# stevenrobertson/cuburn

Measured on AMD Instinct MI355X. Metric: Msamples/s into 1920x1080 histogram + DE-filter GB/s vs HBM roofline, higher is better.
Workload: dtype f32; 1 GPU; BASELINE configs[1]: 1920x1080 still, 3 xforms (linear+spherical+swirl), 2^28 samples/frame, filters yuv+bilateral+logscale+colorclip, rgba8 out; walker_waves=4, walker_slots=1024, temporal_samples=1024, samples_per_frame=268435456, accum=binned, fuse=256, nslots=1024, frames_queued_ahead=2, frames_per_gpu=1121, parallelism=frame-sharded x1, RCCL gather of device frames, 4 frames per collective

## Files before the change

cuburn_amd/_lib.py:

```python
import ctypes as C
import os

_HERE = os.path.dirname(os.path.abspath(__file__))
LIB_PATH = os.path.join(_HERE, '_lib', 'libflame_hip.so')
LIB_PATH = os.environ.get('FLAME_HIP_LIB', LIB_PATH)

(FL_OK, FL_E_INVAL, FL_E_NOMEM, FL_E_HIP, FL_E_NODEV, FL_E_UNSUPPORTED) = (0, -1, -2, -3, -4, -5)

FILT = dict(yuv=0, bilateral=1, logscale=2, colorclip=3, smearclip=4, haloclip=5, plainclip=6, logencode=7, de=8)
BUF = dict(front=0, back=1, params=2, palette=3, points=4, seeds=5, atom=6, hot=7, side=8)
ACCUM_ATOMIC, ACCUM_BINNED = 0, 1
FL_OP_OPACITY = 10
OUT = dict(rgba8=0, rgba16=1, yuv444p=2, yuv444p10=3, yuv420p10=4, yuv444p12=5)


class fl_dim(C.Structure):
    _fields_ = [(n, C.c_uint32) for n in ('w', 'h', 'aw', 'ah', 'astride')]


_SIGS = {
    'fl_abi_version': (C.c_int, []),
    'fl_last_error': (C.c_char_p, []),
    'fl_calc_dim': (None, [C.c_uint32, C.c_uint32, C.POINTER(fl_dim)]),
    'fl_ctx_create': (C.c_int, [C.c_int, C.c_void_p, C.c_void_p, C.c_uint32, C.c_uint32, C.POINTER(C.c_void_p)]),
    'fl_ctx_destroy': (None, [C.c_void_p]),
    'fl_ctx_sync': (C.c_int, [C.c_void_p]),
    'fl_genome_create': (C.c_int, [C.c_void_p, C.c_void_p, C.c_uint32, C.c_void_p, C.c_uint32, C.c_uint32,
                                   C.POINTER(C.c_void_p)]),
    'fl_genome_destroy': (None, [C.c_void_p]),
    'fl_genome_upload': (C.c_int, [C.c_void_p, C.c_void_p, C.c_void_p, C.c_void_p, C.c_void_p, C.c_void_p, C.c_uint32]),
    'fl_interp': (C.c_int, [C.c_void_p, C.c_void_p, C.c_uint32, C.c_uint32, C.c_float, C.c_float]),
    'fl_iterate': (C.c_int, [C.c_void_p, C.c_void_p, C.c_uint32, C.c_uint32, C.c_double, C.c_uint32, C.c_int,
                             C.POINTER(C.c_uint64)]),
    'fl_filter': (C.c_int, [C.c_void_p, C.c_int, C.c_uint32, C.c_uint32, C.c_void_p, C.c_uint32]),
    'fl_output': (C.c_int, [C.c_void_p, C.c_uint32, C.c_uint32, C.c_int, C.c_void_p, C.c_uint64]),
    'fl_output_bytes': (C.c_size_t, [C.c_uint32, C.c_uint32, C.c_int]),
    'fl_sort_u32': (C.c_int, [C.c_void_p, C.c_uint64, C.c_uint64, C.c_uint32, C.c_uint32, C.c_uint32, C.c_int, C.c_void_p]),
    'fl_frame_begin': (C.c_int, [C.c_void_p, C.POINTER(C.c_uint32)]),
    'fl_frame_ms': (C.c_int, [C.c_void_p, C.c_uint32, C.POINTER(C.c_float)]),
    'fl_frame_query': (C.c_int, [C.c_void_p, C.c_uint32]),
    'fl_host_alloc': (C.c_void_p, [C.c_size_t]),
    'fl_host_free': (None, [C.c_void_p]),
    'fl_timings_reset': (C.c_int, [C.c_void_p]),
    'fl_timings': (C.c_int, [C.c_void_p, C.POINTER(C.c_float), C.POINTER(C.c_float), C.POINTER(C.c_float),
                             C.POINTER(C.c_uint32)]),
    'fl_timings_detail': (C.c_int, [C.c_void_p, C.POINTER(C.c_float * 6)]),
    'fl_launch_stats': (C.c_int, [C.c_void_p, C.POINTER(C.c_uint32 * 4)]),
    'fl_measure_copy': (C.c_int, [C.c_int, C.c_size_t, C.c_int, C.POINTER(C.c_float)]),
    'fl_read_buffer': (C.c_int, [C.c_void_p, C.c_void_p, C.c_int, C.c_void_p, C.c_size_t]),
    'fl_write_buffer': (C.c_int, [C.c_void_p, C.c_void_p, C.c_int, C.c_void_p, C.c_size_t]),
    'fl_buffer_ptr': (C.c_int, [C.c_void_p, C.c_void_p, C.c_int, C.POINTER(C.c_void_p), C.POINTER(C.c_size_t)]),
    'fl_buffer_ptr_async': (C.c_int, [C.c_void_p, C.c_void_p, C.c_int, C.POINTER(C.c_void_p), C.POINTER(C.c_size_t)]),
    'fl_stream_dependency': (C.c_int, [C.c_void_p, C.c_void_p, C.c_int]),
    'fl_reserve': (C.c_int, [C.c_void_p, C.c_uint32, C.c_uint32]),
    'fl_debug_iter_launch': (C.c_int, [C.c_void_p, C.c_void_p, C.c_uint32, C.c_uint32, C.c_uint32, C.c_uint32,
                                       C.c_uint32, C.c_int]),
    'fl_debug_flush': (C.c_int, [C.c_void_p, C.c_uint32, C.c_uint32]),
    'fl_debug_clear': (C.c_int, [C.c_void_p, C.c_uint32, C.c_uint32, C.c_int]),
    'fl_debug_clear_hot': (C.c_int, [C.c_void_p, C.c_uint32, C.c_uint32]),
    'fl_debug_shuffle': (C.c_int, [C.c_void_p, C.c_uint32, C.c_void_p]),
    'fl_debug_counters': (C.c_int, [C.c_void_p, C.c_void_p]),
    'fl_rtc_compile_check': (C.c_int, [C.c_void_p, C.c_uint32, C.c_void_p, C.c_uint32, C.c_int, C.c_int, C.c_int, C.c_char_p, C.c_size_t]),
    'fl_debug_apply_xf': (C.c_int, [C.c_void_p, C.c_void_p, C.c_uint32, C.c_int, C.c_uint32, C.c_void_p, C.c_void_p]),
}
EXPORTS = sorted(_SIGS)

_lib = None


class FlameError(RuntimeError):
    pass


def load():
    global _lib
    if _lib is not None:
        return _lib
    if not os.path.isfile(LIB_PATH):
        raise FlameError('%s not found: build it with `python __graft_entry__.py` '
                         '(make -C cuburn_amd/csrc); the HIP library is required' % LIB_PATH)
    try:
        import torch
    except Exception:
        pass
    lib = C.CDLL(LIB_PATH, mode=C.RTLD_GLOBAL)
    for name, (res, args) in _SIGS.items():
        fn = getattr(lib, name)
        fn.restype, fn.argtypes = res, args
    if lib.fl_abi_version() != 1:
        raise FlameError('libflame_hip ABI mismatch')
    _lib = lib
    return lib


def check(rc):
    if rc == FL_OK:
        return
    msg = load().fl_last_error().decode('utf-8', 'replace')
    if rc == FL_E_NOMEM:
        raise MemoryError(msg)
    if rc in (FL_E_INVAL, FL_E_UNSUPPORTED):
        raise ValueError(msg)
    raise FlameError(msg)
```

cuburn_amd/csrc/flame_abi.hip:

```cpp
#include <hip/hip_runtime.h>
#include <cstdio>
#include <cstdlib>
#include <cstring>
#include <cmath>
#include <string>
#include <atomic>
#include <vector>
#include <algorithm>
#include "kernels.h"
#include "flame_device.h"

static thread_local std::string g_err;
static int fail(int code, const char *what, const char *file, int line, hipError_t e = hipSuccess)
{
    char buf[512];
    if (e != hipSuccess) snprintf(buf, sizeof buf, "%s: %s (%s:%d)", what, hipGetErrorString(e), file, line);
    else snprintf(buf, sizeof buf, "%s (%s:%d)", what, file, line);
    g_err = buf;
    return code;
}
#define HIPCHK(x) do { hipError_t e_ = (x); if (e_ != hipSuccess) \
    return fail(e_ == hipErrorOutOfMemory ? FL_E_NOMEM : FL_E_HIP, #x, __FILE__, __LINE__, e_); } while (0)
#define REQUIRE(c, msg) do { if (!(c)) return fail(FL_E_INVAL, msg, __FILE__, __LINE__); } while (0)

struct EvPair { hipEvent_t a, b; };

struct Lane {
    hipStream_t stream = nullptr;
    size_t nbins = 0;
    float4 *d_front = nullptr, *d_back = nullptr, *d_side = nullptr;
    float *d_blur = nullptr;
    u64 *d_atom = nullptr;
    uint32_t *d_hot = nullptr;
    void *d_outpix = nullptr;
    uint32_t *d_de_tmax = nullptr;
    float *d_de_sinv = nullptr;
    size_t outpix_bytes = 0;
    uint32_t *d_log[2] = {nullptr, nullptr}, *d_dir[2] = {nullptr, nullptr};
    size_t log_words[2] = {0, 0}, dir_words[2] = {0, 0};
    hipStream_t aux = nullptr;
    hipEvent_t ev_it[2] = {nullptr, nullptr}, ev_ac[2] = {nullptr, nullptr};
    float *d_params = nullptr;
    uint64_t params_serial = 0;
    size_t params_floats = 0;
    u64 *d_palette = nullptr;
    hipEvent_t ev_interp_done = nullptr;
    hipEvent_t ev_iter_done = nullptr;
    hipEvent_t ev_out_done = nullptr;
    bool interp_rec = false, iter_rec = false, out_rec = false;
    bool pend_yuv = false, pend_finish = false, pend_log = false;
    float pend_k1 = 0.0f, pend_k2 = 0.0f;
    int pend_in_mode = 0;
    float pend_dp[5] = {0, 0, 0, 0, 0}, pend_k7[7] = {0, 0, 0, 0, 0, 0, 0};
    fl_dim pend_dim = {0, 0, 0, 0, 0};
};

struct fl_ctx {
    int device = 0;
    bool own_stream = false;
    static const int kMaxLanes = 4;
    int nlanes = 2, cur = 0;
    Lane lanes[kMaxLanes];
    uint32_t nslots = 0, nwalkers = 0;
    uint32_t sub_log2 = 0;
    uint32_t ntemporal() const { return nslots << sub_log2; }
    int nw = 4;
    fl_mwc *d_rng = nullptr;
    float4 *d_points = nullptr;
    u64 *d_counters = nullptr;
    uint32_t *d_sort = nullptr; size_t sort_words = 0;
    uint32_t bin_rounds = 16, bin_parts = 0;
    uint32_t launch_rounds = 0;
    uint32_t round_counter = 0;
    static const uint32_t kFrames = 8;
    hipEvent_t ev_begin_[kFrames] = {}, ev_end_[kFrames] = {};
    uint32_t frame_lane[kFrames] = {};
    uint32_t frame_seq = 0;
    std::vector<EvPair> pool, iter_ev, accum_ev, flush_ev, filt_ev, de_ev;
    size_t pool_used = 0;
    bool timing = true;
    static const uint32_t kDepEvents = 16;
    hipEvent_t dep_ev[kDepEvents] = {};
    uint32_t dep_next = 0;
    bool env_bin_wide = false, env_no_intra = false;
    bool use_rtc = true;
    uint32_t n_spec_launch = 0, n_interp_launch = 0;
};
#define L(c) ((c)->lanes[(c)->cur])
#define OTHER(c) ((c)->lanes[((c)->cur + (c)->nlanes - 1) % (c)->nlanes])
#define FL_NOUT 65536u

struct fl_genome {
    uint64_t serial = 0;
    std::vector<int32_t> prog;
    IterSpec spec;
    hipFunction_t rtc_fn[5][2][4] = {};
    unsigned rtc_epoch = 0;
    bool rtc_failed = false;
    uint32_t nops = 0, nrows = 0, pstride = 0;
    int32_t *d_prog = nullptr, *d_ops = nullptr;
    float *d_times = nullptr, *d_knots = nullptr, *d_ptimes = nullptr;
    float4 *d_pals = nullptr;
    uint32_t npal = 0;
    static const int kStage = 4;
    unsigned char *h_stage[kStage] = {};
    hipEvent_t ev_stage[kStage] = {};
    size_t stage_bytes = 0;
    int stage_next = 0;
};

static const int kKnownVars[] = {0,1,2,3,4,5,6,7,8,9,10,11,12,13,14,15,16,17,18,19,20,21,22,23,24,25,26,27,28,29,30,31,32,33,
    34,35,36,37,38,39,40,41,42,43,44,45,46,48,49,50,51,52,53,54,55,56,57,58,59,60,61,62,63,64,65,66,67,68,69,70,71,72,73,
    74,75,76,77,80,81,82,83,84,85,86,87,88,89,90,91,92,93,94,95,97,98};

static const size_t kMaxTimed = 8192;

static EvPair *ev_begin(fl_ctx *c, std::vector<EvPair> &list)
{
    if (!c->timing || c->pool_used >= kMaxTimed) return nullptr;
    if (c->pool.capacity() < kMaxTimed) c->pool.reserve(kMaxTimed);
    if (c->pool_used == c->pool.size()) {
        EvPair p;
        if (hipEventCreate(&p.a) != hipSuccess || hipEventCreate(&p.b) != hipSuccess) return nullptr;
        c->pool.push_back(p);
    }
    EvPair p = c->pool[c->pool_used++];
    list.push_back(p);
    hipEventRecord(p.a, L(c).stream);
    return &c->pool[c->pool_used - 1];
}
static EvPair *ev_pair(fl_ctx *c, std::vector<EvPair> &list)
{
    if (!c->timing || c->pool_used >= kMaxTimed) return nullptr;
    if (c->pool.capacity() < kMaxTimed) c->pool.reserve(kMaxTimed);
    if (c->pool_used == c->pool.size()) {
        EvPair p;
        if (hipEventCreate(&p.a) != hipSuccess || hipEventCreate(&p.b) != hipSuccess) return nullptr;
        c->pool.push_back(p);
    }
    list.push_back(c->pool[c->pool_used++]);
    return &c->pool[c->pool_used - 1];
}
static void ev_end(fl_ctx *c, EvPair *p) { if (p) hipEventRecord(p->b, L(c).stream); }
static EvPair *ev_begin_on(fl_ctx *c, std::vector<EvPair> &list, hipStream_t st)
{
    EvPair *p = ev_pair(c, list);
    if (p) hipEventRecord(p->a, st);
    return p;
}
static void ev_end_on(EvPair *p, hipStream_t st) { if (p) hipEventRecord(p->b, st); }

#pragma GCC visibility push(default)
extern "C" {

int fl_abi_version(void) { return FL_ABI_VERSION; }
const char *fl_last_error(void) { return g_err.c_str(); }

void fl_calc_dim(uint32_t w, uint32_t h, fl_dim *o)
{
    o->w = w; o->h = h;
    o->aw = w + 2 * FL_GUTTER;
    o->ah = 16 * ((h + 2 * FL_GUTTER + 15) / 16);
    o->astride = 32 * ((o->aw + 31) / 32);
}

static void flush_pending(fl_ctx *c);

static const float *de_norms()
{
    static const std::vector<float> t = [] { std::vector<float> v(16 * FL_DE_MAX_RADIUS + 1); de_adaptive_norms(v.data()); return v; }();
    return t.data();
}

static void free_fb(fl_ctx *c)
{
    hipFree(L(c).d_front); hipFree(L(c).d_back); hipFree(L(c).d_side); hipFree(L(c).d_blur);
    hipFree(L(c).d_atom); hipFree(L(c).d_hot); hipFree(L(c).d_outpix); hipFree(L(c).d_de_tmax); hipFree(L(c).d_de_sinv);
    L(c).d_front = L(c).d_back = L(c).d_side = nullptr; L(c).d_blur = nullptr; L(c).d_atom = nullptr;
    L(c).d_hot = nullptr; L(c).d_outpix = nullptr; L(c).d_de_tmax = nullptr; L(c).d_de_sinv = nullptr;
    L(c).nbins = 0; L(c).outpix_bytes = 0;
    L(c).pend_yuv = L(c).pend_finish = L(c).pend_log = false;
}

static int ensure_fb(fl_ctx *c, const fl_dim &d)
{
    size_t nbins = (size_t)d.ah * d.astride, ob = (size_t)d.w * d.h * 8;
    if (L(c).nbins >= nbins && L(c).outpix_bytes >= ob) return FL_OK;
    hipStreamSynchronize(L(c).stream);
    free_fb(c);
    hipError_t e;
    if ((e = hipMalloc(&L(c).d_front, 16 * nbins)) || (e = hipMalloc(&L(c).d_back, 16 * nbins)) ||
        (e = hipMalloc(&L(c).d_side, 16 * nbins)) || (e = hipMalloc(&L(c).d_blur, 4 * nbins)) ||
        (e = hipMalloc(&L(c).d_atom, 8 * nbins)) || (e = hipMalloc(&L(c).d_hot, 4 * (nbins / 16))) ||
        (e = hipMalloc(&L(c).d_outpix, ob)) ||
        (e = hipMalloc(&L(c).d_de_tmax, 4 * (nbins / 256 + 64))) ||
        (e = hipMalloc(&L(c).d_de_sinv, 4 * (16 * FL_DE_MAX_RADIUS + 1))) ||
        (e = hipMemcpyAsync(L(c).d_de_sinv, de_norms(), 4 * (16 * FL_DE_MAX_RADIUS + 1), hipMemcpyHostToDevice, L(c).stream))) {
        free_fb(c);
        (void)hipGetLastError();
        return fail(e == hipErrorOutOfMemory ? FL_E_NOMEM : FL_E_HIP, "framebuffer allocation", __FILE__, __LINE__, e);
    }
    L(c).nbins = nbins; L(c).outpix_bytes = ob;
    return FL_OK;
}

static bool env_on(const char *name) { const char *e = getenv(name); return e && *e && strcmp(e, "0") != 0; }

int fl_ctx_create(int device, void *stream, const fl_mwc *seeds, uint32_t nseeds, uint32_t nslots, fl_ctx **out)
{
    REQUIRE(out && seeds, "null argument");
    REQUIRE((nslots >= FL_NTEMPORAL || nslots == FL_NTEMPORAL / 2 || nslots == FL_NTEMPORAL / 4) && nslots % 256 == 0 && nslots <= 16384,
            "nslots must be a multiple of 256 in [1024, 16384] (or 512 slots of 8 waves / 256 of 16: two / four temporal samples per workgroup)");
    int ndev = 0;
    if (hipGetDeviceCount(&ndev) != hipSuccess || ndev <= 0) return fail(FL_E_NODEV, "no HIP device", __FILE__, __LINE__);
    REQUIRE(device >= 0 && device < ndev, "bad device index");
    HIPCHK(hipSetDevice(device));
    hipDeviceProp_t prop;
    HIPCHK(hipGetDeviceProperties(&prop, device));
    if (strncmp(prop.gcnArchName, "gfx950", 6) != 0)
        return fail(FL_E_NODEV, "device is not gfx950 (kernels are built for MI355X only)", __FILE__, __LINE__);
    int nw = 0;
    {
        const uint32_t fixed = FL_PAL_H * 256 + FL_NOUT;
        const uint32_t per_wave = nslots * 64u;
        if (nseeds == fixed + 16u * per_wave) nw = 16;
        else if (nseeds == fixed + 8u * per_wave) nw = 8;
        else if (nseeds == fixed + 4u * per_wave) nw = 4;
        else return fail(FL_E_INVAL, "nseeds must be nslots*64*NW + 64*256 + 65536 with NW = 4, 8 or 16", __FILE__, __LINE__);
    }
    fl_ctx *c = new fl_ctx;
    c->device = device;
    c->nw = nw;
    if (nslots < FL_NTEMPORAL && (uint32_t)nw * nslots != 4u * FL_NTEMPORAL)
        return fail(FL_E_INVAL, "512 slots need 8-wave workgroups, 256 slots 16-wave ones (a temporal sample per four waves: 1024 in all)", __FILE__, __LINE__);
    c->nslots = nslots;
    c->sub_log2 = nslots >= FL_NTEMPORAL ? 0u : nw == 8 ? 1u : 2u;
    c->nwalkers = nslots * (uint32_t)nw * 64 + FL_PAL_H * 256 + FL_NOUT;
    if (const char *e = getenv("FLAME_LANES")) { const int v = atoi(e); c->nlanes = v >= 1 && v <= fl_ctx::kMaxLanes ? v : 2; }
    if (const char *e = getenv("FLAME_BIN_ROUNDS")) { int v = atoi(e); if (v >= 1 && v <= FL_BIN_R_MAX) c->bin_rounds = (uint32_t)v; }
    if (const char *e = getenv("FLAME_BIN_PARTS")) { int v = atoi(e); if (v >= 1 && v <= 64) c->bin_parts = (uint32_t)v; }
    c->env_bin_wide = env_on("FLAME_BIN_WIDE");
    if (const char *e = getenv("FLAME_RTC")) c->use_rtc = strcmp(e, "0") != 0;
    c->env_no_intra = env_on("FLAME_NO_INTRA_OVERLAP");
    if (const char *e = getenv("FLAME_LAUNCH_ROUNDS")) { int v = atoi(e); if (v >= 16 && v <= 4096) c->launch_rounds = (uint32_t)(v / 16 * 16); }
    if (stream) { c->lanes[0].stream = (hipStream_t)stream; c->own_stream = false; c->nlanes = 1; }
    else c->own_stream = true;
    hipError_t e = hipSuccess;
    const char *what = "context allocation";
    do {
        if (c->own_stream)
            for (int i = 0; i < c->nlanes && e == hipSuccess; ++i) e = hipStreamCreateWithFlags(&c->lanes[i].stream, hipStreamNonBlocking);
        if (e) break;
        if ((e = hipMalloc(&c->d_rng, sizeof(fl_mwc) * (size_t)c->nwalkers))) break;
        if ((e = hipMalloc(&c->d_points, sizeof(float4) * (size_t)nslots * nw * 64))) break;
        if ((e = hipMalloc(&c->d_counters, 8 * 4))) break;
        for (int i = 0; i < c->nlanes && e == hipSuccess; ++i) {
            Lane &ln = c->lanes[i];
            if ((e = hipMalloc(&ln.d_palette, sizeof(u64) * FL_PAL_H * FL_PAL_W))) break;
            if ((e = hipEventCreateWithFlags(&ln.ev_interp_done, hipEventDisableTiming))) break;
            if ((e = hipEventCreateWithFlags(&ln.ev_iter_done, hipEventDisableTiming))) break;
            if ((e = hipEventCreateWithFlags(&ln.ev_out_done, hipEventDisableTiming))) break;
            if ((e = hipStreamCreateWithFlags(&ln.aux, hipStreamNonBlocking))) break;
            for (int k = 0; k < 2 && e == hipSuccess; ++k) {
                if ((e = hipEventCreateWithFlags(&ln.ev_it[k], hipEventDisableTiming))) break;
                e = hipEventCreateWithFlags(&ln.ev_ac[k], hipEventDisableTiming);
            }
            if (e) break;
        }
        if (e) break;
        if ((e = hipMemcpy(c->d_rng, seeds, sizeof(fl_mwc) * (size_t)c->nwalkers, hipMemcpyHostToDevice))) break;
        if ((e = hipMemsetD32(c->d_points, 0x7fc00000, (size_t)nslots * nw * 64 * 4))) break;
        if ((e = hipMemset(c->d_counters, 0, 32))) break;
        for (uint32_t i = 0; i < fl_ctx::kFrames && e == hipSuccess; ++i) {
            if ((e = hipEventCreate(&c->ev_begin_[i]))) break;
            e = hipEventCreate(&c->ev_end_[i]);
        }
    } while (0);
    if (e != hipSuccess) {
        fl_ctx_destroy(c);
        (void)hipGetLastError();
        return fail(e == hipErrorOutOfMemory ? FL_E_NOMEM : FL_E_HIP, what, __FILE__, __LINE__, e);
    }
    *out = c;
    return FL_OK;
}

static void sync_all(fl_ctx *c)
{
    for (int i = 0; i < c->nlanes; ++i) { hipStreamSynchronize(c->lanes[i].stream); if (c->lanes[i].aux) hipStreamSynchronize(c->lanes[i].aux); }
}

void fl_ctx_destroy(fl_ctx *c)
{
    if (!c) return;
    hipSetDevice(c->device);
    for (uint32_t i = 0; i < fl_ctx::kDepEvents; ++i) if (c->dep_ev[i]) hipEventDestroy(c->dep_ev[i]);
    for (int i = 0; i < fl_ctx::kMaxLanes; ++i) {
        if (c->lanes[i].stream) hipStreamSynchronize(c->lanes[i].stream);
        if (c->lanes[i].aux) hipStreamSynchronize(c->lanes[i].aux);
    }
    for (int i = 0; i < fl_ctx::kMaxLanes; ++i) {
        c->cur = i;
        free_fb(c);
        Lane &ln = c->lanes[i];
        hipFree(ln.d_params); hipFree(ln.d_palette);
        for (int k = 0; k < 2; ++k) {
            hipFree(ln.d_log[k]); hipFree(ln.d_dir[k]);
            if (ln.ev_it[k]) hipEventDestroy(ln.ev_it[k]);
            if (ln.ev_ac[k]) hipEventDestroy(ln.ev_ac[k]);
        }
        if (ln.aux) hipStreamDestroy(ln.aux);
        if (ln.ev_interp_done) hipEventDestroy(ln.ev_interp_done);
        if (ln.ev_iter_done) hipEventDestroy(ln.ev_iter_done);
        if (ln.ev_out_done) hipEventDestroy(ln.ev_out_done);
        if (c->own_stream && ln.stream) hipStreamDestroy(ln.stream);
    }
    hipFree(c->d_rng); hipFree(c->d_points); hipFree(c->d_counters); hipFree(c->d_sort);
    for (auto &p : c->pool) { hipEventDestroy(p.a); hipEventDestroy(p.b); }
    for (uint32_t i = 0; i < fl_ctx::kFrames; ++i) {
        if (c->ev_begin_[i]) hipEventDestroy(c->ev_begin_[i]);
        if (c->ev_end_[i]) hipEventDestroy(c->ev_end_[i]);
    }
    (void)hipGetLastError();
    delete c;
}

int fl_ctx_sync(fl_ctx *c) { REQUIRE(c, "null ctx"); sync_all(c); return FL_OK; }

static int wait_other(fl_ctx *c, int what)
{
    if (c->nlanes < 2) return FL_OK;
    Lane &o = OTHER(c);
    if (what == 0 && o.interp_rec) HIPCHK(hipStreamWaitEvent(L(c).stream, o.ev_interp_done, 0));
    if (what == 1 && o.iter_rec) HIPCHK(hipStreamWaitEvent(L(c).stream, o.ev_iter_done, 0));
    if (what == 2 && o.out_rec) HIPCHK(hipStreamWaitEvent(L(c).stream, o.ev_out_done, 0));
    return FL_OK;
}

static int check_prog(const int32_t *p, uint32_t n)
{
    REQUIRE(n >= FL_PROG_HDR && p[0] == FL_PROG_MAGIC, "bad program header");
    int nxf = p[1], hf = p[2], ps = p[3], cdf = p[4], xo = p[5], xs = p[6], vs = p[7];
    REQUIRE(nxf >= 1 && nxf <= FL_MAX_XFORMS && (hf == 0 || hf == 1), "bad xform count");
    REQUIRE(ps >= 6 + nxf && ps <= FL_MAX_PSTRIDE, "bad pstride");
    REQUIRE(cdf >= 6 && cdf + nxf <= xo, "bad cdf offset");
    REQUIRE(xs >= FL_XF_HDR + vs && (xs % 4) == 0 && vs >= 2 && vs <= 64, "bad record strides");
    REQUIRE(xo + (nxf + hf) * xs <= ps, "xform records exceed the block");
    return FL_OK;
}

static bool known_var(int id)
{
    for (int k : kKnownVars) if (k == id) return true;
    return false;
}

int fl_genome_create(fl_ctx *c, const int32_t *prog, uint32_t nprog, const int32_t *ops, uint32_t nops,
                     uint32_t nrows, fl_genome **out)
{
    REQUIRE(c && prog && ops && out, "null argument");
    int rc = check_prog(prog, nprog);
    if (rc) return rc;
    REQUIRE(nrows >= 1 && nrows <= 4096 && nops >= 1, "bad row / op count");
    uint32_t ps = prog[3];
    const int xo = prog[5], xs = prog[6], vs = prog[7], nrec = prog[1] + prog[2];
    std::vector<int> nvar_seen(nrec, -1), opac_seen(nrec, 0), opac_ops(nrec, 0);
    for (uint32_t i = 0; i < nops; ++i) {
        const int32_t *o = ops + 4 * i;
        REQUIRE(o[0] >= FL_OP_SPLINE && o[0] <= FL_OP_OPACITY, "bad op kind");
        REQUIRE(o[1] >= 0 && (uint32_t)o[1] < ps, "op destination out of range");
        if (o[0] != FL_OP_CONST) {
            uint32_t ndst = 1, nsrc = 1;
            switch (o[0]) {
            case FL_OP_CAMERA: ndst = 6; nsrc = 4; break;
            case FL_OP_AFFINE: ndst = 6; nsrc = 6; break;
            case FL_OP_CDF:
                REQUIRE(o[3] >= 1 && o[3] <= FL_MAX_XFORMS, "bad CDF length");
                ndst = nsrc = (uint32_t)o[3];
                break;
            case FL_OP_PERSP: ndst = 3; break;
            default: break;
            }
            REQUIRE((uint32_t)o[1] + ndst <= ps, "op destination out of range");
            REQUIRE(o[2] >= 0 && (uint32_t)o[2] + nsrc <= nrows, "op row out of range");
            if (o[0] == FL_OP_RATIO2 || o[0] == FL_OP_PERSP) REQUIRE(o[3] >= 0 && (uint32_t)o[3] < nrows, "op row out of range");
            if (o[0] == FL_OP_OPACITY) {
                const int rel = o[1] - xo;
                REQUIRE(rel >= 0 && rel / xs < prog[1] && rel % xs == 15, "opacity op must write word 15 of a selectable xform record");
                ++opac_ops[rel / xs];
            }
            continue;
        }
        const int rel = o[1] - xo;
        REQUIRE(rel >= 0 && rel / xs < nrec, "structure word outside the xform records");
        const int w = rel % xs;
        if (w == 14) {
            const int nv = o[2] & 0xff;
            REQUIRE(FL_XF_HDR + nv * vs <= xs && (o[2] >> 10) == 0, "bad variation count");
            REQUIRE(((o[2] >> 9) & 1) == 0 || rel / xs < prog[1], "the final xform has no opacity");
            nvar_seen[rel / xs] = nv;
            opac_seen[rel / xs] = (o[2] >> 9) & 1;
        } else {
            REQUIRE(w >= FL_XF_HDR && (w - FL_XF_HDR) % vs == 0, "misplaced structure word");
            if (!known_var(o[2])) return fail(FL_E_UNSUPPORTED, "unknown variation id", __FILE__, __LINE__);
        }
    }
    for (int i = 0; i < nrec; ++i) REQUIRE(nvar_seen[i] >= 0, "xform record without a variation count");
    for (int i = 0; i < nrec; ++i) REQUIRE(opac_ops[i] == opac_seen[i], "opacity flag and opacity op do not match");
    IterSpec spec;
    spec.nxf = prog[1]; spec.has_final = prog[2]; spec.pstride = prog[3]; spec.cdf_off = prog[4];
    spec.xf_off = xo; spec.xf_stride = xs; spec.var_stride = vs;
    spec.nvar.assign(nrec, 0); spec.post.assign(nrec, 0); spec.opac.assign(nrec, 0); spec.vids.assign(nrec, std::vector<int>());
    for (int i = 0; i < nrec; ++i) spec.vids[i].assign(nvar_seen[i], -1);
    for (uint32_t i = 0; i < nops; ++i) {
        const int32_t *o = ops + 4 * i;
        if (o[0] != FL_OP_CONST) continue;
        const int rel = o[1] - xo, rec = rel / xs, w = rel % xs;
        if (w == 14) { spec.nvar[rec] = o[2] & 0xff; spec.post[rec] = (o[2] >> 8) & 1; spec.opac[rec] = (o[2] >> 9) & 1; }
        else {
            const int j = (w - FL_XF_HDR) / vs;
            if (j < (int)spec.vids[rec].size()) spec.vids[rec][j] = o[2];
        }
    }
    for (int i = 0; i < nrec; ++i)
        for (int v : spec.vids[i]) REQUIRE(v >= 0, "variation record without a variation number");
    HIPCHK(hipSetDevice(c->device));
    fl_genome *g = new fl_genome;
    { static std::atomic<uint64_t> next_serial{1}; g->serial = next_serial.fetch_add(1); }
    g->spec = spec;
    g->prog.assign(prog, prog + nprog);
    g->nops = nops; g->nrows = nrows; g->pstride = ps;
    g->stage_bytes = 2 * 4 * (size_t)nrows * FL_KNOTS + 16 * 256 * (FL_KNOTS - 1) + 4 * FL_KNOTS;
    hipError_t e = hipSuccess;
    do {
        if ((e = hipMalloc(&g->d_prog, 4 * nprog))) break;
        if ((e = hipMalloc(&g->d_ops, 16 * nops))) break;
        if ((e = hipMalloc(&g->d_times, 4 * (size_t)nrows * FL_KNOTS))) break;
        if ((e = hipMalloc(&g->d_knots, 4 * (size_t)nrows * FL_KNOTS))) break;
        if ((e = hipMalloc(&g->d_ptimes, 4 * FL_KNOTS))) break;
        if ((e = hipMalloc(&g->d_pals, 16 * 256 * FL_KNOTS))) break;
        if ((e = hipMemcpy(g->d_prog, prog, 4 * nprog, hipMemcpyHostToDevice))) break;
        if ((e = hipMemcpy(g->d_ops, ops, 16 * nops, hipMemcpyHostToDevice))) break;
        if ((e = hipMemset(g->d_pals, 0, 16 * 256 * FL_KNOTS))) break;
        for (int i = 0; i < fl_genome::kStage && e == hipSuccess; ++i) {
            if ((e = hipHostMalloc((void **)&g->h_stage[i], g->stage_bytes, hipHostMallocDefault))) break;
            e = hipEventCreateWithFlags(&g->ev_stage[i], hipEventDisableTiming);
        }
    } while (0);
    if (e != hipSuccess) {
        fl_genome_destroy(g);
        (void)hipGetLastError();
        return fail(e == hipErrorOutOfMemory ? FL_E_NOMEM : FL_E_HIP, "genome allocation", __FILE__, __LINE__, e);
    }
    *out = g;
    return FL_OK;
}

void fl_genome_destroy(fl_genome *g)
{
    if (!g) return;
    hipFree(g->d_prog); hipFree(g->d_ops); hipFree(g->d_times); hipFree(g->d_knots);
    hipFree(g->d_ptimes); hipFree(g->d_pals);
    for (int i = 0; i < fl_genome::kStage; ++i) { if (g->h_stage[i]) hipHostFree(g->h_stage[i]); if (g->ev_stage[i]) hipEventDestroy(g->ev_stage[i]); }
    delete g;
}

int fl_genome_upload(fl_ctx *c, fl_genome *g, const float *times, const float *knots,
                     const float *pal_rgba, const float *pal_times, uint32_t npal)
{
    REQUIRE(c && g && times && knots && pal_rgba && pal_times, "null argument");
    REQUIRE(npal >= 1 && npal < FL_KNOTS, "bad palette count");
    HIPCHK(hipSetDevice(c->device));
    const size_t nb = 4 * (size_t)g->nrows * FL_KNOTS, pb = 16 * 256 * (size_t)npal, tb = 4 * FL_KNOTS;
    const int slot = g->stage_next;
    g->stage_next = (slot + 1) % fl_genome::kStage;
    HIPCHK(hipEventSynchronize(g->ev_stage[slot]));
    unsigned char *h = g->h_stage[slot];
    memcpy(h, times, nb);
    memcpy(h + nb, knots, nb);
    memcpy(h + 2 * nb, pal_rgba, pb);
    memcpy(h + 2 * nb + pb, pal_times, tb);
    { int rc = wait_other(c, 0); if (rc) return rc; }
    HIPCHK(hipMemcpyAsync(g->d_times, h, nb, hipMemcpyHostToDevice, L(c).stream));
    HIPCHK(hipMemcpyAsync(g->d_knots, h + nb, nb, hipMemcpyHostToDevice, L(c).stream));
    HIPCHK(hipMemcpyAsync(g->d_pals, h + 2 * nb, pb, hipMemcpyHostToDevice, L(c).stream));
    HIPCHK(hipMemcpyAsync(g->d_ptimes, h + 2 * nb + pb, tb, hipMemcpyHostToDevice, L(c).stream));
    HIPCHK(hipEventRecord(g->ev_stage[slot], L(c).stream));
    g->npal = npal;
    return FL_OK;
}

int fl_frame_begin(fl_ctx *c, uint32_t *frame_id)
{
    REQUIRE(c && frame_id, "null argument");
    HIPCHK(hipSetDevice(c->device));
    const uint32_t id = c->frame_seq++;
    const uint32_t k = id % fl_ctx::kFrames;
    c->cur = (int)(id % (uint32_t)c->nlanes);
    c->frame_lane[k] = (uint32_t)c->cur;
    HIPCHK(hipEventRecord(c->ev_begin_[k], L(c).stream));
    HIPCHK(hipEventRecord(c->ev_end_[k], L(c).stream));
    *frame_id = id;
    return FL_OK;
}

int fl_interp(fl_ctx *c, fl_genome *g, uint32_t w, uint32_t h, float ts, float td)
{
    REQUIRE(c && g && g->npal, "genome not uploaded");
    HIPCHK(hipSetDevice(c->device));
    fl_dim d; fl_calc_dim(w, h, &d);
    const size_t need = (size_t)c->ntemporal() * g->pstride;
    if (need > L(c).params_floats) {
        HIPCHK(hipStreamSynchronize(L(c).stream));
        hipFree(L(c).d_params); L(c).d_params = nullptr; L(c).params_floats = 0;
        HIPCHK(hipMalloc(&L(c).d_params, sizeof(float) * need));
        L(c).params_floats = need; L(c).params_serial = 0;
    }
    fl_mwc *rng_pal = c->d_rng + (size_t)c->nslots * c->nw * 64;
    { int rc = wait_other(c, 0); if (rc) return rc; }
    launch_interp_palette(L(c).stream, rng_pal, g->d_ptimes, g->d_pals, ts, td / FL_PAL_H, L(c).d_palette);
    launch_interp_params(L(c).stream, L(c).d_params, g->d_times, g->d_knots, g->d_ops, g->nops, g->pstride,
                         c->ntemporal(), ts, td / (float)c->ntemporal(), d, L(c).params_serial != g->serial);
    L(c).params_serial = g->serial;
    HIPCHK(hipGetLastError());
    HIPCHK(hipEventRecord(L(c).ev_interp_done, L(c).stream));
    L(c).interp_rec = true;
    return FL_OK;
}

static int do_clear(fl_ctx *c, const fl_dim &d, bool reset_points)
{
    size_t nbins = (size_t)d.ah * d.astride;
    launch_clear_frame(L(c).stream, L(c).d_front, L(c).d_atom, L(c).d_hot, c->d_counters, c->d_points, (uint32_t)nbins,
                       reset_points ? c->nslots * (uint32_t)c->nw * 64u : 0u);
    HIPCHK(hipGetLastError());
    return FL_OK;
}

#define FL_BIN_MAX_ROUNDS 1024u
#define FL_BIN_MAX_ROUNDS_LONG 2304u

static int ensure_binned(fl_ctx *c, const fl_dim &d, uint32_t write_rounds, int buf, uint32_t *tiles_x, uint32_t *nbins,
                         uint32_t *nbatch_total, bool *wide)
{
    const uint32_t nt = (uint32_t)c->nw * 64;
    const uint32_t rows = (d.ah + FL_TILE_H - 1) / FL_TILE_H;
    *wide = ((d.astride + 127) / 128) * rows > FL_MAX_BINS || c->env_bin_wide;
    const uint32_t tw = *wide ? (1u << FL_TILE_W_WIDE_LOG2) : 128u;
    *tiles_x = (d.astride + tw - 1) / tw;
    *nbins = *tiles_x * rows;
    if (*nbins > FL_MAX_BINS_WIDE) return fail(FL_E_UNSUPPORTED, "image too large for the binned accumulate (> 8191 tiles of 256x64)", __FILE__, __LINE__);
    const uint32_t per_slot = (write_rounds + c->bin_rounds - 1) / c->bin_rounds;
    *nbatch_total = per_slot * c->nslots;
    const size_t region = !*wide && FL_LOG_PACK3 ? 2 * (size_t)fl_pack3_words(c->bin_rounds * nt) : (size_t)c->bin_rounds * nt;
    size_t lw = (size_t)*nbatch_total * region + 8, dw = (size_t)*nbins * *nbatch_total;
    if (lw > L(c).log_words[buf]) {
        HIPCHK(hipStreamSynchronize(L(c).stream)); HIPCHK(hipStreamSynchronize(L(c).aux));
        hipFree(L(c).d_log[buf]); L(c).d_log[buf] = nullptr; L(c).log_words[buf] = 0;
        HIPCHK(hipMalloc(&L(c).d_log[buf], lw * 4));
        L(c).log_words[buf] = lw;
    }
    if (dw > L(c).dir_words[buf]) {
        HIPCHK(hipStreamSynchronize(L(c).stream)); HIPCHK(hipStreamSynchronize(L(c).aux));
        hipFree(L(c).d_dir[buf]); L(c).d_dir[buf] = nullptr; L(c).dir_words[buf] = 0;
        HIPCHK(hipMalloc(&L(c).d_dir[buf], dw * 4));
        L(c).dir_words[buf] = dw;
    }
    return FL_OK;
}

static int do_iter_launch(fl_ctx *c, fl_genome *g, const fl_dim &d, uint32_t nrounds, uint32_t fuse, bool count, int acc = 0,
                          int buf = 0, hipStream_t drain = nullptr)
{
    if (!drain) drain = L(c).stream;
    uint32_t tiles_x = 0, nbins = 0, nbatch_total = 0;
    bool wide = false;
    if (acc == FL_ACCUM_BINNED) {
        if (nrounds <= fuse) return fail(FL_E_INVAL, "binned launch needs write-enabled rounds", __FILE__, __LINE__);
        int rc = ensure_binned(c, d, nrounds - fuse, buf, &tiles_x, &nbins, &nbatch_total, &wide);
        if (rc) return rc;
    }
    EvPair *e = ev_pair(c, c->iter_ev);
    const int kacc = acc == FL_ACCUM_BINNED && wide ? 3 : acc;
    hipFunction_t fn = nullptr;
    if (c->use_rtc && !g->rtc_failed && kacc != 2) {
        const unsigned ep = rtc_epoch();
        if (g->rtc_epoch != ep) { memset(g->rtc_fn, 0, sizeof g->rtc_fn); g->rtc_epoch = ep; }
        hipFunction_t &slot = g->rtc_fn[c->sub_log2 ? 2 + c->sub_log2 : c->nw == 16 ? 2 : c->nw == 8][count ? 1 : 0][kacc];
        if (!slot) {
            std::string err;
            if (rtc_iter_kernel(c->device, g->spec, c->nw, c->nslots, count, kacc, &slot, &err, c->sub_log2)) {
                g->rtc_failed = true;
                slot = nullptr;
                fprintf(stderr, "libflame_hip: per-genome kernel not available (%s); using the interpreter kernel\n", err.c_str());
            }
        }
        fn = slot;
    }
    (fn ? c->n_spec_launch : c->n_interp_launch) += 1;
    if (fn)
        launch_iter_fn(L(c).stream, fn, c->nw, kacc, c->nslots, g->d_prog, L(c).d_params, L(c).d_palette, c->d_rng, c->d_points,
                       L(c).d_hot, L(c).d_atom, (float *)L(c).d_front, c->d_counters, d.astride, d.ah, c->round_counter, nrounds, fuse,
                       tiles_x, nbins, c->bin_rounds, nbatch_total, L(c).d_log[buf], L(c).d_dir[buf],
                       e ? e->a : nullptr, e ? e->b : nullptr, c->sub_log2);
    else
    launch_iter(L(c).stream, c->nw, count, kacc, c->nslots, g->d_prog, L(c).d_params, L(c).d_palette, c->d_rng, c->d_points,
                L(c).d_hot, L(c).d_atom, (float *)L(c).d_front, c->d_counters, d.astride, d.ah, c->round_counter, nrounds, fuse,
                tiles_x, nbins, c->bin_rounds, nbatch_total, L(c).d_log[buf], L(c).d_dir[buf],
                e ? e->a : nullptr, e ? e->b : nullptr, c->sub_log2);
    c->round_counter += nrounds;
    HIPCHK(hipGetLastError());
    if (acc == FL_ACCUM_BINNED) {
        if (drain != L(c).stream) {
            HIPCHK(hipEventRecord(L(c).ev_it[buf], L(c).stream));
            HIPCHK(hipStreamWaitEvent(drain, L(c).ev_it[buf], 0));
        }
        EvPair *e2 = ev_begin_on(c, c->accum_ev, drain);
        uint32_t parts = c->bin_parts ? c->bin_parts : nbins > 512u ? ((wide ? 12800u : 6400u) + nbins / 2u) / nbins : (wide ? 16384u : 8192u) / nbins;
        parts = parts < 1u ? 1u : parts > (c->bin_parts ? 64u : 16u) ? (c->bin_parts ? 64u : 16u) : parts;
        launch_accum_tiles(drain, L(c).d_log[buf], L(c).d_dir[buf], L(c).d_palette, L(c).d_atom, (float *)L(c).d_front, tiles_x, nbins,
                           parts, nbatch_total, c->bin_rounds * (uint32_t)c->nw * 64, c->nslots, d.astride, d.ah, wide);
        ev_end_on(e2, drain);
        HIPCHK(hipGetLastError());
    }
    return FL_OK;
}

static int do_flush(fl_ctx *c, const fl_dim &d, bool use_hot = true, hipStream_t st = nullptr)
{
    if (!st) st = L(c).stream;
    EvPair *e = ev_begin_on(c, c->flush_ev, st);
    launch_flush(st, L(c).d_atom, L(c).d_front, L(c).d_hot, d.ah * d.astride, use_hot);
    ev_end_on(e, st);
    HIPCHK(hipGetLastError());
    return FL_OK;
}

int fl_iterate(fl_ctx *c, fl_genome *g, uint32_t w, uint32_t h, double nsamples, uint32_t fuse,
               int accum_mode, uint64_t *nsamples_run)
{
    REQUIRE(c && g, "null argument");
    REQUIRE(accum_mode == FL_ACCUM_ATOMIC || accum_mode == FL_ACCUM_BINNED || accum_mode == 2, "bad accumulation mode");
    REQUIRE(L(c).params_floats >= (size_t)c->ntemporal() * g->pstride, "fl_interp has not run for this genome");
    HIPCHK(hipSetDevice(c->device));
    fl_dim d; fl_calc_dim(w, h, &d);
    int rc = ensure_fb(c, d);
    if (rc) return rc;
    flush_pending(c);
    if ((rc = wait_other(c, 1))) return rc;
    if ((rc = do_clear(c, d, true))) return rc;
    const uint32_t nt = (uint32_t)c->nw * 64;
    const double per_round = (double)c->nslots * nt;
    uint64_t rounds = (uint64_t)ceil(nsamples / per_round);
    if (rounds == 0) rounds = 1;
    if (nsamples_run) *nsamples_run = (uint64_t)(rounds * per_round);
    const uint64_t unit = 256ull << c->sub_log2;
    auto launches_with = [rounds, unit](uint64_t cap_) { uint32_t nl = 0; for (uint64_t r = rounds, b = 4; r; b += b / 2) { r -= std::min(std::min(r, b * unit), cap_); ++nl; } return nl; };
    const uint64_t cap_short = (uint64_t)FL_BIN_MAX_ROUNDS << c->sub_log2;
    uint64_t cap_long = (uint64_t)(c->nw == 16 ? 1536u : FL_BIN_MAX_ROUNDS_LONG) << c->sub_log2;
    if (accum_mode == FL_ACCUM_BINNED && !c->launch_rounds && launches_with(cap_long) < launches_with(cap_short)) {
        const uint32_t nt_ = (uint32_t)c->nw * 64;
        const bool wide_ = ((d.astride + 127) / 128) * ((d.ah + FL_TILE_H - 1) / FL_TILE_H) > FL_MAX_BINS || c->env_bin_wide;
        const uint32_t tw_ = wide_ ? (1u << FL_TILE_W_WIDE_LOG2) : 128u;
        const size_t nbins_ = (size_t)((d.astride + tw_ - 1) / tw_) * ((d.ah + FL_TILE_H - 1) / FL_TILE_H);
        const size_t region = !wide_ && FL_LOG_PACK3 ? 2 * (size_t)fl_pack3_words(c->bin_rounds * nt_) : (size_t)c->bin_rounds * nt_;
        const size_t nb_long = (size_t)((std::min(rounds, cap_long) + c->bin_rounds - 1) / c->bin_rounds) * c->nslots;
        const size_t need = (nb_long * region + 8 + nbins_ * nb_long) * 4;
        size_t have = 0, grow = 0;
        for (int b = 0; b < 2; ++b) {
            have = (L(c).log_words[b] + L(c).dir_words[b]) * 4;
            if (need > have) grow += need - have;
        }
        size_t mfree = 0, mtotal = 0;
        if (grow && (hipMemGetInfo(&mfree, &mtotal) != hipSuccess || grow + (size_t(1) << 30) > mfree)) cap_long = cap_short;
    }
    const uint64_t cap = accum_mode != FL_ACCUM_BINNED ? ~0ull : c->launch_rounds ? c->launch_rounds :
                         launches_with(cap_long) < launches_with(cap_short) ? cap_long : cap_short;
    const uint32_t nlaunch = launches_with(cap);
    const bool pipelined = accum_mode == FL_ACCUM_BINNED && nlaunch > 1 && !c->env_no_intra;
    hipStream_t drain = pipelined ? L(c).aux : L(c).stream;
    uint64_t batch = 4;
    uint32_t k = 0;
    while (rounds) {
        const uint64_t n = std::min(std::min(rounds, batch * unit), cap);
        const uint32_t f = k == 0 ? fuse : 0;
        const int buf = pipelined ? (int)(k & 1u) : 0;
        if (pipelined && k >= 2) HIPCHK(hipStreamWaitEvent(L(c).stream, L(c).ev_ac[buf], 0));
        if ((rc = do_iter_launch(c, g, d, (uint32_t)n + f, f, false, accum_mode, buf, drain))) return rc;
        if ((rc = do_flush(c, d, accum_mode != FL_ACCUM_BINNED, drain))) return rc;
        if (pipelined) HIPCHK(hipEventRecord(L(c).ev_ac[buf], drain));
        rounds -= n;
        batch += batch / 2;
        ++k;
    }
    HIPCHK(hipEventRecord(L(c).ev_iter_done, L(c).stream));
    L(c).iter_rec = true;
    if (pipelined) {
        HIPCHK(hipStreamWaitEvent(L(c).stream, L(c).ev_ac[(k - 1) & 1u], 0));
        if (k >= 2) HIPCHK(hipStreamWaitEvent(L(c).stream, L(c).ev_ac[k & 1u], 0));
    }
    return FL_OK;
}

static void gauss7(float stdev, float *c)
{
    float s = 0.0f;
    for (int i = 0; i < 7; ++i) { float x = (float)(i - 3); c[i] = expf(x * x / (-2.0f * stdev * stdev)); s += c[i]; }
    for (int i = 0; i < 7; ++i) c[i] /= s;
}

static void run_de_finish(fl_ctx *c, const float *clip)
{
    Lane &ln = L(c);
    DeTail t = {ln.pend_log ? 1 : 0, ln.pend_k1, ln.pend_k2, clip ? 1 : 0, clip ? clip[0] : 0.f, clip ? clip[1] : 0.f,
                clip ? clip[2] : 0.f, clip ? clip[3] : 0.f, clip ? clip[4] : 0.f};
    EvPair *e = ev_begin(c, c->de_ev);
    float4 *Na = ln.d_back, *Nb = ln.d_front;
    launch_de_dir(ln.stream, ln.pend_dim, 0, Na, Nb, ln.pend_k7, ln.pend_dp[0], ln.pend_dp[1], ln.pend_dp[2], ln.pend_dp[3], ln.pend_dp[4], ln.pend_in_mode, nullptr);
    for (int pat = 1; pat < 7; ++pat) {
        launch_de_dir(ln.stream, ln.pend_dim, pat, Nb, Na, ln.pend_k7, ln.pend_dp[0], ln.pend_dp[1], ln.pend_dp[2], ln.pend_dp[3], ln.pend_dp[4]);
        std::swap(Na, Nb);
    }
    launch_de_dir(ln.stream, ln.pend_dim, 7, ln.d_front, Na, ln.pend_k7, ln.pend_dp[0], ln.pend_dp[1], ln.pend_dp[2], ln.pend_dp[3], ln.pend_dp[4], 0, &t);
    ev_end(c, e);
    ln.pend_finish = ln.pend_log = false;
}

static void flush_pending(fl_ctx *c)
{
    Lane &ln = L(c);
    if (ln.pend_yuv) {
        launch_yuv_to_rgb(ln.stream, ln.pend_dim, ln.d_back, ln.d_front);
        std::swap(ln.d_front, ln.d_back);
        ln.pend_yuv = false;
    }
    if (ln.pend_finish) run_de_finish(c, nullptr);
}

int fl_filter(fl_ctx *c, int id, uint32_t w, uint32_t h, const float *p, uint32_t np)
{
    REQUIRE(c, "null ctx");
    HIPCHK(hipSetDevice(c->device));
    fl_dim d; fl_calc_dim(w, h, &d);
    int rc = ensure_fb(c, d);
    if (rc) return rc;
    hipStream_t st = L(c).stream;
    float k7[7];
    EvPair *e = ev_begin(c, c->filt_ev);
    switch (id) {
    case FL_FILT_YUV:
        flush_pending(c);
        L(c).pend_yuv = true; L(c).pend_dim = d;
        break;
    case FL_FILT_BILATERAL: {
        REQUIRE(np >= 5, "bilateral needs sstd,cstd,dstd,dpow,gspeed");
        gauss7(1.0f, k7);
        if (L(c).pend_finish) flush_pending(c);
        L(c).pend_in_mode = L(c).pend_yuv ? 2 : 1;
        L(c).pend_yuv = false;
        L(c).pend_finish = true; L(c).pend_log = false; L(c).pend_dim = d;
        for (int i = 0; i < 5; ++i) L(c).pend_dp[i] = p[i];
        for (int i = 0; i < 7; ++i) L(c).pend_k7[i] = k7[i];
    } break;
    case FL_FILT_LOGSCALE:
        REQUIRE(np >= 2, "logscale needs k1,k2");
        if (L(c).pend_finish && !L(c).pend_log && !L(c).pend_yuv) { L(c).pend_log = true; L(c).pend_k1 = p[0]; L(c).pend_k2 = p[1]; break; }
        flush_pending(c);
        launch_logscale(st, d, L(c).d_front, p[0], p[1]);
        break;
    case FL_FILT_COLORCLIP:
        REQUIRE(np >= 5, "colorclip needs vib,highpow,gam,lin,lingam");
        if (L(c).pend_finish && !L(c).pend_yuv) {
            run_de_finish(c, p);
            break;
        }
        flush_pending(c);
        launch_colorclip(st, d, L(c).d_front, p[0], p[1], p[2], p[3], p[4]);
        break;
    case FL_FILT_SMEARCLIP:
        flush_pending(c);
        REQUIRE(np >= 4, "smearclip needs width,gam_m_1,lin,lingam");
        gauss7(p[0], k7);
        launch_gamma_full_hi(st, d, L(c).d_side, L(c).d_front);
        launch_full_blur(st, d, L(c).d_back, L(c).d_side, 2, 0, k7);
        launch_full_blur(st, d, L(c).d_side, L(c).d_back, 3, 0, k7);
        launch_full_blur(st, d, L(c).d_back, L(c).d_side, 0, 0, k7);
        launch_full_blur(st, d, L(c).d_side, L(c).d_back, 1, 0, k7);
        launch_smearclip(st, d, L(c).d_front, L(c).d_side, p[1], p[2], p[3]);
        break;
    case FL_FILT_HALOCLIP:
        flush_pending(c);
        REQUIRE(np >= 1, "haloclip needs gam_m_1");
        gauss7(1.0f, k7);
        launch_apply_gamma(st, d, L(c).d_blur, L(c).d_front, 0.1f);
        launch_den_blur_1c(st, d, (float *)L(c).d_side, L(c).d_blur, 2, 0, k7);
        launch_den_blur_1c(st, d, L(c).d_blur, (const float *)L(c).d_side, 3, 0, k7);
        launch_haloclip(st, d, L(c).d_front, L(c).d_blur, p[0]);
        break;
    case FL_FILT_PLAINCLIP:
        flush_pending(c);
        REQUIRE(np >= 4, "plainclip needs gam_m_1,lin,lingam,brightness");
        launch_plainclip(st, d, L(c).d_front, p[0], p[1], p[2], p[3]);
        break;
    case FL_FILT_LOGENCODE:
        flush_pending(c);
        REQUIRE(np >= 1, "logencode needs degamma");
        launch_logencode(st, d, L(c).d_back, L(c).d_front, p[0]);
        std::swap(L(c).d_front, L(c).d_back);
        break;
    case FL_FILT_DE: {
        flush_pending(c);
        REQUIRE(np >= 3, "de needs R,Rmin,curve");
        REQUIRE(!(p[0] > (float)FL_DE_MAX_RADIUS), "de: R above 96 px");
        REQUIRE(p[2] > 0.0f, "de: curve must be > 0");
        if (!(p[0] > 0.0f)) break;
        launch_de_adaptive(st, d, L(c).d_front, L(c).d_back, L(c).d_blur, L(c).d_de_tmax, L(c).d_de_sinv,
                           p[0], std::min(std::max(p[1], 0.0f), p[0]), p[2]);
    } break;
    default:
        return fail(FL_E_UNSUPPORTED, "unknown filter id", __FILE__, __LINE__);
    }
    ev_end(c, e);
    HIPCHK(hipGetLastError());
    return FL_OK;
}

size_t fl_output_bytes(uint32_t w, uint32_t h, int fmt)
{
    const size_t n = (size_t)w * h;
    switch (fmt) {
    case FL_OUT_RGBA8: return 4 * n;
    case FL_OUT_RGBA16: return 8 * n;
    case FL_OUT_YUV444P: return 3 * n;
    case FL_OUT_YUV444P10: case FL_OUT_YUV444P12: return 6 * n;
    case FL_OUT_YUV420P10: return 3 * n;
    default: return 0;
    }
}

int fl_output(fl_ctx *c, uint32_t w, uint32_t h, int fmt, void *host_out, uint64_t dev_out)
{
    REQUIRE(c && fl_output_bytes(w, h, fmt) != 0, "bad argument");
    REQUIRE(fmt != FL_OUT_YUV420P10 || (w % 2 == 0 && h % 2 == 0), "4:2:0 needs even width and height");
    HIPCHK(hipSetDevice(c->device));
    fl_dim d; fl_calc_dim(w, h, &d);
    int rc = ensure_fb(c, d);
    if (rc) return rc;
    flush_pending(c);
    void *dst = dev_out ? (void *)(uintptr_t)dev_out : L(c).d_outpix;
    { int rc2 = wait_other(c, 2); if (rc2) return rc2; }
    fl_mwc *rng_out = c->d_rng + (size_t)c->nslots * c->nw * 64 + FL_PAL_H * 256;
    launch_f32_to_rgba(L(c).stream, d, L(c).d_front, rng_out, FL_NOUT, fmt, dst);
    HIPCHK(hipGetLastError());
    HIPCHK(hipEventRecord(L(c).ev_out_done, L(c).stream));
    L(c).out_rec = true;
    if (host_out) HIPCHK(hipMemcpyAsync(host_out, dst, fl_output_bytes(w, h, fmt), hipMemcpyDeviceToHost, L(c).stream));
    if (c->frame_seq) HIPCHK(hipEventRecord(c->ev_end_[(c->frame_seq - 1) % fl_ctx::kFrames], L(c).stream));
    return FL_OK;
}

int fl_sort_u32(fl_ctx *c, uint64_t dst_dev, uint64_t src_dev, uint32_t n, uint32_t lo_bit, uint32_t nbits, int ignore_max,
                uint32_t *nvalid)
{
    REQUIRE(c && dst_dev && src_dev && dst_dev != src_dev, "null or aliased key arrays");
    REQUIRE(nbits >= 1 && nbits <= 10 && lo_bit + nbits <= 32, "a pass sorts 1..10 bits inside the 32-bit key");
    HIPCHK(hipSetDevice(c->device));
    if (n == 0) { if (nvalid) *nvalid = 0; return FL_OK; }
    size_t chunk_words = 0;
    const size_t hist_words = sort_scratch_words(n, nbits, &chunk_words), need = hist_words + chunk_words;
    hipStream_t sst = c->lanes[0].stream;
    if (need > c->sort_words) {
        sync_all(c);
        hipFree(c->d_sort); c->d_sort = nullptr; c->sort_words = 0;
        HIPCHK(hipMalloc(&c->d_sort, need * 4));
        c->sort_words = need;
    }
    uint32_t *chunk_tot = c->d_sort + hist_words, *total_dev = chunk_tot + (chunk_words - 1);
    launch_sort_pass(sst, (uint32_t *)(uintptr_t)dst_dev, (const uint32_t *)(uintptr_t)src_dev, n, lo_bit, nbits,
                     ignore_max, c->d_sort, chunk_tot, total_dev);
    HIPCHK(hipGetLastError());
    if (nvalid) {
        HIPCHK(hipMemcpyAsync(nvalid, total_dev, 4, hipMemcpyDeviceToHost, sst));
        HIPCHK(hipStreamSynchronize(sst));
    }
    return FL_OK;
}

int fl_frame_ms(fl_ctx *c, uint32_t frame_id, float *ms)
{
    REQUIRE(c && ms, "null argument");
    REQUIRE(frame_id < c->frame_seq && c->frame_seq - frame_id <= fl_ctx::kFrames, "frame id no longer tracked");
    const uint32_t k = frame_id % fl_ctx::kFrames;
    HIPCHK(hipEventSynchronize(c->ev_end_[k]));
    HIPCHK(hipEventElapsedTime(ms, c->ev_begin_[k], c->ev_end_[k]));
    return FL_OK;
}

int fl_frame_query(fl_ctx *c, uint32_t frame_id)
{
    REQUIRE(c, "null ctx");
    REQUIRE(frame_id < c->frame_seq && c->frame_seq - frame_id <= fl_ctx::kFrames, "frame id no longer tracked");
    hipError_t e = hipEventQuery(c->ev_end_[frame_id % fl_ctx::kFrames]);
    if (e == hipSuccess) return 1;
    if (e == hipErrorNotReady) { (void)hipGetLastError(); return 0; }
    return fail(FL_E_HIP, "hipEventQuery", __FILE__, __LINE__, e);
}

void *fl_host_alloc(size_t nbytes)
{
    void *p = nullptr;
    if (hipHostMalloc(&p, nbytes, hipHostMallocDefault) != hipSuccess) { (void)hipGetLastError(); return nullptr; }
    return p;
}

void fl_host_free(void *p) { if (p) hipHostFree(p); }

static float sum_ms(std::vector<EvPair> &v)
{
    float t = 0.0f;
    for (auto &p : v) { float ms = 0.0f; if (hipEventElapsedTime(&ms, p.a, p.b) == hipSuccess) t += ms; }
    return t;
}

int fl_timings_reset(fl_ctx *c)
{
    REQUIRE(c, "null ctx");
    sync_all(c);
    c->iter_ev.clear(); c->accum_ev.clear(); c->flush_ev.clear(); c->filt_ev.clear(); c->de_ev.clear(); c->pool_used = 0;
    c->n_spec_launch = c->n_interp_launch = 0;
    return FL_OK;
}

int fl_timings_detail(fl_ctx *c, float ms[6])
{
    REQUIRE(c && ms, "null argument");
    sync_all(c);
    ms[0] = sum_ms(c->iter_ev); ms[1] = sum_ms(c->accum_ev); ms[2] = sum_ms(c->flush_ev);
    ms[3] = sum_ms(c->filt_ev); ms[4] = sum_ms(c->de_ev); ms[5] = 0.0f;
    return FL_OK;
}

int fl_launch_stats(fl_ctx *c, uint32_t out[4])
{
    REQUIRE(c && out, "null argument");
    out[0] = c->n_spec_launch; out[1] = c->n_interp_launch; out[2] = c->nslots; out[3] = (uint32_t)c->nw;
    return FL_OK;
}

int fl_measure_copy(int device, size_t nbytes, int iters, float *ms)
{
    REQUIRE(ms && iters > 0 && nbytes >= 16, "bad argument");
    HIPCHK(hipSetDevice(device));
    if (launch_measure_copy(nbytes, iters, ms)) return fail(FL_E_HIP, "copy measurement (allocation of 2 x nbytes, or the launch)", __FILE__, __LINE__);
    return FL_OK;
}

int fl_timings(fl_ctx *c, float *iter_ms, float *flush_ms, float *filter_ms, uint32_t *nlaunch)
{
    REQUIRE(c, "null ctx");
    sync_all(c);
    if (iter_ms) *iter_ms = sum_ms(c->iter_ev);
    if (flush_ms) *flush_ms = sum_ms(c->accum_ev) + sum_ms(c->flush_ev);
    if (filter_ms) *filter_ms = sum_ms(c->filt_ev);
    if (nlaunch) *nlaunch = (uint32_t)c->iter_ev.size();
    return FL_OK;
}

static int buf_ptr(fl_ctx *c, fl_genome *g, int which, void **p, size_t *cap)
{
    switch (which) {
    case FL_BUF_FRONT: *p = L(c).d_front; *cap = 16 * L(c).nbins; break;
    case FL_BUF_BACK: *p = L(c).d_back; *cap = 16 * L(c).nbins; break;
    case FL_BUF_SIDE: *p = L(c).d_side; *cap = 16 * L(c).nbins; break;
    case FL_BUF_PARAMS: *p = L(c).d_params; *cap = 4 * L(c).params_floats; break;
    case FL_BUF_PALETTE: *p = L(c).d_palette; *cap = 8 * FL_PAL_H * FL_PAL_W; break;
    case FL_BUF_POINTS: *p = c->d_points; *cap = 16 * (size_t)c->nslots * c->nw * 64; break;
    case FL_BUF_SEEDS: *p = c->d_rng; *cap = sizeof(fl_mwc) * (size_t)c->nwalkers; break;
    case FL_BUF_ATOM: *p = L(c).d_atom; *cap = 8 * L(c).nbins; break;
    case FL_BUF_HOT: *p = L(c).d_hot; *cap = 4 * (L(c).nbins / 16); break;
    default: return fail(FL_E_INVAL, "unknown buffer", __FILE__, __LINE__);
    }
    if (!*p) return fail(FL_E_INVAL, "buffer not allocated yet", __FILE__, __LINE__);
    return FL_OK;
}

int fl_read_buffer(fl_ctx *c, fl_genome *g, int which, void *dst, size_t nbytes)
{
    REQUIRE(c && dst, "null argument");
    HIPCHK(hipSetDevice(c->device));
    flush_pending(c);
    void *p; size_t cap;
    int rc = buf_ptr(c, g, which, &p, &cap);
    if (rc) return rc;
    REQUIRE(nbytes <= cap, "read larger than buffer");
    sync_all(c);
    HIPCHK(hipMemcpy(dst, p, nbytes, hipMemcpyDeviceToHost));
    return FL_OK;
}

int fl_buffer_ptr(fl_ctx *c, fl_genome *g, int which, void **dev_ptr, size_t *nbytes)
{
    REQUIRE(c && dev_ptr && nbytes, "null argument");
    HIPCHK(hipSetDevice(c->device));
    flush_pending(c);
    int rc = buf_ptr(c, g, which, dev_ptr, nbytes);
    if (rc) return rc;
    sync_all(c);
    return FL_OK;
}

int fl_buffer_ptr_async(fl_ctx *c, fl_genome *g, int which, void **dev_ptr, size_t *nbytes)
{
    REQUIRE(c && dev_ptr && nbytes, "null argument");
    HIPCHK(hipSetDevice(c->device));
    flush_pending(c);
    return buf_ptr(c, g, which, dev_ptr, nbytes);
}

int fl_reserve(fl_ctx *c, uint32_t w, uint32_t h)
{
    REQUIRE(c && w && h, "bad argument");
    HIPCHK(hipSetDevice(c->device));
    fl_dim d; fl_calc_dim(w, h, &d);
    return ensure_fb(c, d);
}

int fl_stream_dependency(fl_ctx *c, void *stream, int ctx_waits)
{
    REQUIRE(c, "null ctx");
    HIPCHK(hipSetDevice(c->device));
    hipStream_t other = (hipStream_t)stream;
    hipEvent_t &ev = c->dep_ev[c->dep_next++ % fl_ctx::kDepEvents];
    if (!ev) HIPCHK(hipEventCreateWithFlags(&ev, hipEventDisableTiming));
    if (ctx_waits) {
        HIPCHK(hipEventRecord(ev, other));
        HIPCHK(hipStreamWaitEvent(L(c).stream, ev, 0));
    } else {
        flush_pending(c);
        HIPCHK(hipEventRecord(ev, L(c).stream));
        HIPCHK(hipStreamWaitEvent(other, ev, 0));
    }
    return FL_OK;
}

int fl_write_buffer(fl_ctx *c, fl_genome *g, int which, const void *src, size_t nbytes)
{
    REQUIRE(c && src, "null argument");
    HIPCHK(hipSetDevice(c->device));
    flush_pending(c);
    void *p; size_t cap;
    int rc = buf_ptr(c, g, which, &p, &cap);
    if (rc) return rc;
    REQUIRE(nbytes <= cap, "write larger than buffer");
    sync_all(c);
    HIPCHK(hipMemcpy(p, src, nbytes, hipMemcpyHostToDevice));
    if (which == FL_BUF_PARAMS) L(c).params_serial = 0;
    return FL_OK;
}

int fl_debug_clear(fl_ctx *c, uint32_t w, uint32_t h, int reset_points)
{
    REQUIRE(c, "null ctx");
    HIPCHK(hipSetDevice(c->device));
    fl_dim d; fl_calc_dim(w, h, &d);
    int rc = ensure_fb(c, d);
    if (rc) return rc;
    flush_pending(c);
    return do_clear(c, d, reset_points != 0);
}

int fl_debug_iter_launch(fl_ctx *c, fl_genome *g, uint32_t w, uint32_t h, uint32_t round0,
                         uint32_t nrounds, uint32_t fuse, int accum_mode)
{
    REQUIRE(c && g && (accum_mode == FL_ACCUM_ATOMIC || accum_mode == FL_ACCUM_BINNED), "bad argument");
    REQUIRE(L(c).params_floats >= (size_t)c->ntemporal() * g->pstride, "fl_interp has not run for this genome");
    HIPCHK(hipSetDevice(c->device));
    fl_dim d; fl_calc_dim(w, h, &d);
    int rc = ensure_fb(c, d);
    if (rc) return rc;
    c->round_counter = round0;
    HIPCHK(hipMemsetAsync(c->d_counters, 0, 32, L(c).stream));
    return do_iter_launch(c, g, d, nrounds, fuse, true, accum_mode);
}

int fl_debug_flush(fl_ctx *c, uint32_t w, uint32_t h)
{
    REQUIRE(c, "null ctx");
    fl_dim d; fl_calc_dim(w, h, &d);
    int rc = ensure_fb(c, d);
    if (rc) return rc;
    flush_pending(c);
    return do_flush(c, d);
}

int fl_debug_clear_hot(fl_ctx *c, uint32_t w, uint32_t h)
{
    REQUIRE(c && L(c).d_hot, "null ctx");
    fl_dim d; fl_calc_dim(w, h, &d);
    HIPCHK(hipMemsetAsync(L(c).d_hot, 0, 4 * ((size_t)d.ah * d.astride / 16), L(c).stream));
    return FL_OK;
}

struct DevBuf {
    void *p = nullptr;
    ~DevBuf() { if (p) hipFree(p); }
    hipError_t alloc(size_t n) { return hipMalloc(&p, n); }
};

int fl_debug_shuffle(fl_ctx *c, uint32_t round, uint32_t *out256)
{
    REQUIRE(c && out256, "null argument");
    HIPCHK(hipSetDevice(c->device));
    DevBuf d; const size_t n = (size_t)c->nw * 64;
    HIPCHK(d.alloc(4 * n));
    launch_shuffle_tap(L(c).stream, c->nw, (uint32_t *)d.p, round);
    HIPCHK(hipStreamSynchronize(L(c).stream));
    HIPCHK(hipMemcpy(out256, d.p, 4 * n, hipMemcpyDeviceToHost));
    return FL_OK;
}

int fl_debug_apply_xf(fl_ctx *c, fl_genome *g, uint32_t ts, int xfi, uint32_t n, float *xyzw, fl_mwc *rng)
{
    REQUIRE(c && g && xyzw && rng && n > 0 && ts < c->ntemporal(), "bad argument");
    REQUIRE(xfi >= 0 && xfi < g->prog[1] + g->prog[2], "xform index out of range");
    REQUIRE(L(c).params_floats >= (size_t)c->ntemporal() * g->pstride, "fl_interp has not run for this genome");
    HIPCHK(hipSetDevice(c->device));
    DevBuf dp, dr;
    HIPCHK(dp.alloc(16 * (size_t)n));
    HIPCHK(dr.alloc(sizeof(fl_mwc) * (size_t)n));
    HIPCHK(hipMemcpy(dp.p, xyzw, 16 * (size_t)n, hipMemcpyHostToDevice));
    HIPCHK(hipMemcpy(dr.p, rng, sizeof(fl_mwc) * (size_t)n, hipMemcpyHostToDevice));
    launch_apply_xf_tap(L(c).stream, g->d_prog, L(c).d_params, ts, xfi, n, (float4 *)dp.p, (fl_mwc *)dr.p);
    HIPCHK(hipStreamSynchronize(L(c).stream));
    HIPCHK(hipMemcpy(xyzw, dp.p, 16 * (size_t)n, hipMemcpyDeviceToHost));
    HIPCHK(hipMemcpy(rng, dr.p, sizeof(fl_mwc) * (size_t)n, hipMemcpyDeviceToHost));
    return FL_OK;
}

int fl_rtc_compile_check(const int32_t *prog, uint32_t nprog, const int32_t *ops, uint32_t nops, int nw, int count, int acc,
                         char *log, size_t log_bytes)
{
    REQUIRE(prog && ops && nprog >= FL_PROG_HDR && (nw == 4 || nw == 8 || nw == 16) && acc >= 0 && acc <= 3, "bad argument");
    int rc = check_prog(prog, nprog);
    if (rc) return rc;
    const int xo = prog[5], xs = prog[6], vs = prog[7], nrec = prog[1] + prog[2];
    IterSpec spec;
    spec.nxf = prog[1]; spec.has_final = prog[2]; spec.pstride = prog[3]; spec.cdf_off = prog[4];
    spec.xf_off = xo; spec.xf_stride = xs; spec.var_stride = vs;
    spec.nvar.assign(nrec, 0); spec.post.assign(nrec, 0); spec.opac.assign(nrec, 0); spec.vids.assign(nrec, std::vector<int>(16, 0));
    for (uint32_t i = 0; i < nops; ++i) {
        const int32_t *o = ops + 4 * i;
        if (o[0] == FL_OP_OPACITY) {
            const int rel = o[1] - xo;
            REQUIRE(rel >= 0 && rel / xs < prog[1] && rel % xs == 15, "opacity op must write word 15 of a selectable xform record");
        }
        if (o[0] != FL_OP_CONST) continue;
        const int rel = o[1] - xo, rec = rel / xs, w = rel % xs;
        REQUIRE(rel >= 0 && rec < nrec, "structure word outside the xform records");
        if (w == 14) {
            REQUIRE((o[2] >> 10) == 0 && (((o[2] >> 9) & 1) == 0 || rec < prog[1]), "bad structure word");
            spec.nvar[rec] = o[2] & 0xff; spec.post[rec] = (o[2] >> 8) & 1; spec.opac[rec] = (o[2] >> 9) & 1;
        }
        else { const int j = (w - FL_XF_HDR) / vs; if (j >= (int)spec.vids[rec].size()) spec.vids[rec].resize(j + 1, 0); spec.vids[rec][j] = o[2]; }
    }
    std::vector<char> code;
    std::string err;
    rc = rtc_compile(spec, nw, (count & 1) != 0, acc, &code, &err, nullptr, (count & 2) == 0 ? 0u : nw == 8 ? 1u : nw == 16 ? 2u : 0u);
    if (log && log_bytes) { snprintf(log, log_bytes, "%s", rc ? err.c_str() : "ok"); }
    if (rc) return fail(rtc_available() ? FL_E_HIP : FL_E_UNSUPPORTED, "per-genome kernel did not compile", __FILE__, __LINE__);
    return (int)(code.size() > 0 ? FL_OK : FL_E_HIP);
}

int fl_debug_counters(fl_ctx *c, uint64_t out4[4])
{
    REQUIRE(c && out4, "null argument");
    sync_all(c);
    HIPCHK(hipMemcpy(out4, c->d_counters, 32, hipMemcpyDeviceToHost));
    return FL_OK;
}

}
#pragma GCC visibility pop
```

cuburn_amd/csrc/iter.hip:

```cpp
#include "variations.h"
#ifndef FL_RTC
#include "kernels.h"
#include <hip/hip_ext.h>
#endif

#define FL_CNT_SETS 3
#define FL_CNT_SETS_BIG 2
#define FL_SCATTER_DEPTH 4
#ifndef FL_ITER_MERGE_MAX_XF
#define FL_ITER_MERGE_MAX_XF 4
#endif
#ifndef FL_SORT_FULL_COPY
#define FL_SORT_FULL_COPY 1
#endif
#ifndef FL_SORT_LOCAL_TID
#define FL_SORT_LOCAL_TID 1
#endif

template <int NW>
__device__ __forceinline__ uint32_t shuffle_dest(uint32_t w, uint32_t l, uint32_t phase) {
    uint32_t sh = l + (phase == 1 ? l / NW : 0u) + (phase == 2 ? l / (NW * NW) : 0u);
    return ((w + sh) % NW) * 64u + l;
}

struct XfHead { float f[16]; int vid0; float w0; };
#define FL_XTAB_BYTES 256

__device__ __forceinline__ XfHead load_head(const float *__restrict__ xf) {
    XfHead h;
#pragma unroll
    for (int i = 0; i < 16; ++i) h.f[i] = xf[i];
    h.vid0 = __float_as_int(xf[FL_XF_HDR]);
    h.w0 = xf[FL_XF_HDR + 1];
    return h;
}

__device__ __forceinline__ void opacity_mark(const bool has, const float q, float &c, mwc_t &r)
{
    const uint32_t qb = __float_as_uint(q);
    uint32_t hid = 0u;
    if (has) {
        if (qb - 1u < 0x3f800000u - 1u) hid = mwc_next_01(r) <= q ? 0u : 0x80000000u;
        else if (qb == 0u) hid = 0x80000000u;
    }
    c = __uint_as_float((__float_as_uint(c) & 0x7fffffffu) | hid);
}

__device__ __forceinline__ void apply_xf(const XfHead &h, const float *__restrict__ xf, int var_stride,
                                         float &x, float &y, float &c, mwc_t &r, const bool any_opac = false)
{
    const int word14 = __float_as_int(h.f[14]);
    const int nvar = word14 & 0xff;
    float tx = fmaf(h.f[0], x, fmaf(h.f[1], y, h.f[2]));
    float ty = fmaf(h.f[3], x, fmaf(h.f[4], y, h.f[5]));
    float ox = -0.0f, oy = -0.0f;
    if (nvar > 0) apply_variation(h.vid0, h.w0, xf + FL_XF_HDR + 2, xf, tx, ty, ox, oy, r);
    for (int j = 1; j < nvar; ++j) {
        const float *__restrict__ v = xf + FL_XF_HDR + j * var_stride;
        apply_variation(__float_as_int(v[0]), v[1], v + 2, xf, tx, ty, ox, oy, r);
    }
    if (word14 & 0x100) {
        const float qx = fmaf(h.f[6], ox, fmaf(h.f[7], oy, h.f[8]));
        const float qy = fmaf(h.f[9], ox, fmaf(h.f[10], oy, h.f[11]));
        ox = qx; oy = qy;
    }
    const float csp = h.f[13];
    c = fmaf(c, 1.0f - csp, h.f[12] * csp);
    if (any_opac) opacity_mark((word14 & 0x200) != 0, h.f[15], c, r);
    x = ox; y = oy;
}

#ifdef FL_RTC
#include "flame_spec.h"

constexpr int kTailFirst = FL_XF_HDR + 2, kTailWords = 10;
struct XfTail { float w[kTailWords]; };
struct VTail {
    const float *__restrict__ p; const XfTail *t; int base;
    __device__ __forceinline__ float operator[](int i) const {
        const int wd = base + i;
        return (t && wd >= kTailFirst && wd < kTailFirst + kTailWords) ? t->w[wd - kTailFirst] : p[wd];
    }
};
template <int I, int J>
__device__ __forceinline__ void spec_variations(const float *__restrict__ xf, float w0, float &tx, float &ty,
                                                float &ox, float &oy, mwc_t &r, const XfTail *tl = nullptr)
{
    if constexpr (J < kSpecNvar[I]) {
        constexpr int B = FL_XF_HDR + J * FL_SPEC_VAR_STRIDE;
        const VTail v = {xf, tl, B + 2}, vh = {xf, tl, B};
        apply_variation_body(kSpecVid[I][J], J == 0 ? w0 : vh[1], v, xf, tx, ty, ox, oy, r);
        spec_variations<I, J + 1>(xf, w0, tx, ty, ox, oy, r, tl);
    }
}

__host__ __device__ constexpr bool spec_any_opac() { for (int i = 0; i < FL_SPEC_NXF; ++i) if (kSpecOpac[i] != 0) return true; return false; }
constexpr bool kAnyOpac = spec_any_opac();
template <int I>
__device__ __forceinline__ void spec_opacity(const XfHead &h, float &c, mwc_t &r)
{
    if constexpr (kAnyOpac && I < FL_SPEC_NXF) opacity_mark(kSpecOpac[I] != 0, h.f[15], c, r);
}

template <int I>
__device__ __forceinline__ void spec_apply_xf(const XfHead &h, const float *__restrict__ xf,
                                              float &x, float &y, float &c, mwc_t &r)
{
    float tx = fmaf(h.f[0], x, fmaf(h.f[1], y, h.f[2]));
    float ty = fmaf(h.f[3], x, fmaf(h.f[4], y, h.f[5]));
    float ox = -0.0f, oy = -0.0f;
    spec_variations<I, 0>(xf, h.w0, tx, ty, ox, oy, r);
    if constexpr (kSpecPost[I] != 0) {
        const float qx = fmaf(h.f[6], ox, fmaf(h.f[7], oy, h.f[8]));
        const float qy = fmaf(h.f[9], ox, fmaf(h.f[10], oy, h.f[11]));
        ox = qx; oy = qy;
    }
    const float csp = h.f[13];
    c = fmaf(c, 1.0f - csp, h.f[12] * csp);
    spec_opacity<I>(h, c, r);
    x = ox; y = oy;
}

__host__ __device__ constexpr int spec_resident_sgprs()
{
    int n = 0;
    for (int i = 0; i < FL_SPEC_NXF; ++i) n += 9 + (kSpecPost[i] != 0 ? 6 : 0);
    return n;
}
constexpr bool kSpecResident = FL_SPEC_NXF <= 4 && spec_resident_sgprs() <= 48;
#ifndef FL_HOIST_BUDGET
#define FL_HOIST_BUDGET 12
#endif
__host__ __device__ constexpr int spec_npost() { int n = 0; for (int i = 0; i < FL_SPEC_NXF; ++i) n += kSpecPost[i] != 0 ? 1 : 0; return n; }
constexpr bool kHoistCol = kSpecResident && FL_SPEC_NXF + 2 <= FL_HOIST_BUDGET;
constexpr bool kHoistAff = kHoistCol && 3 * FL_SPEC_NXF + 2 <= FL_HOIST_BUDGET;
constexpr bool kHoistPost = kHoistAff && 3 * FL_SPEC_NXF + 2 + 2 * spec_npost() <= FL_HOIST_BUDGET;
struct XfVec { float xo, yo, cprod, pxo, pyo; };
constexpr bool kTab = !kSpecResident && FL_HOIST_BUDGET >= 12 && FL_SPEC_NXF * 16 <= FL_XTAB_BYTES;
template <int I, class Extra>
__device__ __forceinline__ void spec_apply_xf_tab(const XfHead &h, const float4 &t, const float *__restrict__ xf,
                                                  float &x, float &y, float &c, mwc_t &r, const XfTail *tl, Extra &&extra)
{
    extra();
    float tx = fmaf(h.f[0], x, fmaf(h.f[1], y, t.x));
    float ty = fmaf(h.f[3], x, fmaf(h.f[4], y, t.y));
    float ox = -0.0f, oy = -0.0f;
    spec_variations<I, 0>(xf, h.w0, tx, ty, ox, oy, r, tl);
    if constexpr (kSpecPost[I] != 0) {
        const float qx = fmaf(h.f[6], ox, fmaf(h.f[7], oy, h.f[8]));
        const float qy = fmaf(h.f[9], ox, fmaf(h.f[10], oy, h.f[11]));
        ox = qx; oy = qy;
    }
    c = fmaf(c, t.z, t.w);
    asm volatile("" : "+v"(c));
    spec_opacity<I>(h, c, r);
    x = ox; y = oy;
}
template <int LO, int HI, class Extra>
__device__ __forceinline__ void spec_dispatch_tab(int k, const XfHead &h, const float4 &t, const float *__restrict__ xf,
                                                  float &x, float &y, float &c, mwc_t &r, const XfTail *tl, Extra &&extra)
{
    if constexpr (HI - LO == 1) spec_apply_xf_tab<LO>(h, t, xf, x, y, c, r, tl, extra);
    else {
        constexpr int MID = (LO + HI) / 2;
        if (k < MID) spec_dispatch_tab<LO, MID>(k, h, t, xf, x, y, c, r, tl, extra);
        else spec_dispatch_tab<MID, HI>(k, h, t, xf, x, y, c, r, tl, extra);
    }
}
constexpr bool kHoistFinal = FL_SPEC_FINAL != 0 && FL_HOIST_BUDGET >= 7;
template <int I, bool COL = kHoistCol, bool AFF = kHoistAff, bool POST = kHoistPost>
__device__ __forceinline__ void spec_apply_xf_res(const XfHead &h, const XfVec &v, const float *__restrict__ xf,
                                                  float &x, float &y, float &c, mwc_t &r, const XfTail *tl = nullptr)
{
    float tx = fmaf(h.f[0], x, fmaf(h.f[1], y, AFF ? v.xo : h.f[2]));
    float ty = fmaf(h.f[3], x, fmaf(h.f[4], y, AFF ? v.yo : h.f[5]));
    float ox = -0.0f, oy = -0.0f;
    spec_variations<I, 0>(xf, h.w0, tx, ty, ox, oy, r, tl);
    if constexpr (kSpecPost[I] != 0) {
        const float qx = fmaf(h.f[6], ox, fmaf(h.f[7], oy, POST ? v.pxo : h.f[8]));
        const float qy = fmaf(h.f[9], ox, fmaf(h.f[10], oy, POST ? v.pyo : h.f[11]));
        ox = qx; oy = qy;
    }
    if constexpr (COL) { c = fmaf(c, h.f[13], v.cprod); asm volatile("" : "+v"(c)); }
    else { const float csp = h.f[13]; c = fmaf(c, 1.0f - csp, h.f[12] * csp); }
    spec_opacity<I>(h, c, r);
    x = ox; y = oy;
}
template <int LO, int HI, class Extra>
__device__ __forceinline__ void spec_dispatch_res(int k, const XfHead (&heads)[FL_SPEC_NXF], const XfVec (&hv)[FL_SPEC_NXF], const float *__restrict__ xf0, int xf_stride,
                                                  float &x, float &y, float &c, mwc_t &r, const XfTail (&tails)[FL_SPEC_NXF], Extra &&extra)
{
    if constexpr (HI - LO == 1) { extra(); spec_apply_xf_res<LO>(heads[LO], hv[LO], xf0 + LO * xf_stride, x, y, c, r, &tails[LO]); }
    else {
        constexpr int MID = (LO + HI) / 2;
        if (k < MID) spec_dispatch_res<LO, MID>(k, heads, hv, xf0, xf_stride, x, y, c, r, tails, extra);
        else spec_dispatch_res<MID, HI>(k, heads, hv, xf0, xf_stride, x, y, c, r, tails, extra);
    }
}

template <int LO, int HI, class Extra>
__device__ __forceinline__ void spec_dispatch(int k, const XfHead &h, const float *__restrict__ xf,
                                              float &x, float &y, float &c, mwc_t &r, Extra &&extra)
{
    if constexpr (HI - LO == 1) { extra(); spec_apply_xf<LO>(h, xf, x, y, c, r); }
    else {
        constexpr int MID = (LO + HI) / 2;
        if (k < MID) spec_dispatch<LO, MID>(k, h, xf, x, y, c, r, extra);
        else spec_dispatch<MID, HI>(k, h, xf, x, y, c, r, extra);
    }
}
#endif

__device__ __forceinline__ void drain_if_full(bool ok, u64 old, uint32_t gi, float mult,
                                              u64 *__restrict__ atom, float *__restrict__ out4, uint32_t &n_spill)
{
    if (ok && (uint32_t)(old >> 32) >= (256u << 23)) {
        const u64 cur = __hip_atomic_exchange(atom + gi, 0ull, __ATOMIC_RELAXED, __HIP_MEMORY_SCOPE_AGENT);
        if ((uint32_t)(cur >> 32) != 0u) {
            float yf, uf, vf, df;
            unpack_cell(cur, yf, uf, vf, df);
            const float m255 = mult * FL_INV255;
            float *o = out4 + 4 * (size_t)gi;
            __hip_atomic_fetch_add(o + 0, yf * m255, __ATOMIC_RELAXED, __HIP_MEMORY_SCOPE_AGENT);
            __hip_atomic_fetch_add(o + 1, uf * m255, __ATOMIC_RELAXED, __HIP_MEMORY_SCOPE_AGENT);
            __hip_atomic_fetch_add(o + 2, vf * m255, __ATOMIC_RELAXED, __HIP_MEMORY_SCOPE_AGENT);
            __hip_atomic_fetch_add(o + 3, df * mult, __ATOMIC_RELAXED, __HIP_MEMORY_SCOPE_AGENT);
            ++n_spill;
        }
    }
}

__device__ __forceinline__ void reseed(float &x, float &y, float &c, mwc_t &r) {
    x = mwc_next_11(r); y = mwc_next_11(r); c = mwc_next_01(r);
}

struct BinGeom {
    uint32_t tiles_x;
    uint32_t nbins;
    uint32_t rounds;
    uint32_t nbatch_total;
    uint32_t sub_log2;
};

__device__ __forceinline__ uint32_t wave_incl_scan(uint32_t v, uint32_t) {
    v += (uint32_t)__builtin_amdgcn_update_dpp(0, (int)v, 0x111, 0xf, 0xf, false);
    v += (uint32_t)__builtin_amdgcn_update_dpp(0, (int)v, 0x112, 0xf, 0xf, false);
    v += (uint32_t)__builtin_amdgcn_update_dpp(0, (int)v, 0x114, 0xf, 0xf, false);
    v += (uint32_t)__builtin_amdgcn_update_dpp(0, (int)v, 0x118, 0xf, 0xf, false);
    v += (uint32_t)__builtin_amdgcn_update_dpp(0, (int)v, 0x142, 0xa, 0xf, false);
    v += (uint32_t)__builtin_amdgcn_update_dpp(0, (int)v, 0x143, 0xc, 0xf, false);
    return v;
}

template <int NW, bool COUNT, int ACC, bool SPEC>
__device__ __forceinline__ void
iter_body(unsigned char *smem, const int32_t *__restrict__ prog, const float *__restrict__ params,
          const u64 *__restrict__ palette, fl_mwc *__restrict__ rng, float4 *__restrict__ points,
          const uint32_t *__restrict__ hot, u64 *__restrict__ atom, float *__restrict__ out4,
          u64 *__restrict__ counters, uint32_t astride, uint32_t aheight,
          uint32_t round0, uint32_t nrounds, uint32_t fuse, BinGeom bg,
          uint32_t *__restrict__ bin_log, uint32_t *__restrict__ bin_dir)
{
    constexpr int NT = NW * 64;
    constexpr int SETS = NW == 4 ? FL_CNT_SETS : FL_CNT_SETS_BIG;
    constexpr bool BINNED = ACC == 1 || ACC == 3, WIDE = ACC == 3;
    constexpr bool PACK3 = FL_LOG_PACK3 != 0 && ACC == 1;
    constexpr uint32_t TWL = WIDE ? FL_TILE_W_WIDE_LOG2 : 7u;
    constexpr uint32_t PAY_BITS = TWL + FL_TILE_H_LOG2 + 8u;
    float (*swp)[3][NT] = reinterpret_cast<float (*)[3][NT]>(smem);
    u64 *palrow = reinterpret_cast<u64 *>(smem + 2 * 3 * NT * 4);
    uint32_t *stage = reinterpret_cast<uint32_t *>(smem + 2 * 3 * NT * 4);
    uint16_t *skey = reinterpret_cast<uint16_t *>(stage + bg.rounds * NT);
    uint32_t *cnt = stage + bg.rounds * NT + (WIDE ? bg.rounds * NT / 2 : 0);
    const uint32_t CNTW = (bg.nbins + 1 + 3) & ~3u;
    uint32_t *s_nvalid = cnt + SETS * CNTW;
    uint32_t *tot = s_nvalid + 4;
    float4 *xtab = BINNED ? reinterpret_cast<float4 *>(tot + 128) : reinterpret_cast<float4 *>(palrow + FL_PAL_W);
    uint32_t *my_cnt = cnt + ((threadIdx.x & 63u) % SETS) * CNTW;

    const uint32_t tid = threadIdx.x, w = tid >> 6, l = tid & 63;
#ifdef FL_RTC
    constexpr uint32_t kSubSpec = FL_SPEC_SUB_LOG2;
#else
    constexpr uint32_t kSubSpec = 0;
#endif
    const uint32_t sub_log2 = NW == 4 ? 0u : SPEC ? kSubSpec : bg.sub_log2;
    const bool pair = sub_log2 != 0u;
    const uint32_t half = pair ? (uint32_t)__builtin_amdgcn_readfirstlane((int)(w >> 2)) : 0u;
    const uint32_t slot = blockIdx.x, ts = pair ? (slot << sub_log2) + half : slot, prow = slot * FL_PAL_H / gridDim.x;
#ifdef FL_RTC
    const int nxf = SPEC ? FL_SPEC_NXF : prog[1], has_final = SPEC ? FL_SPEC_FINAL : prog[2], pstride = SPEC ? FL_SPEC_PSTRIDE : prog[3];
    const int cdf_off = SPEC ? FL_SPEC_CDF_OFF : prog[4], xf_off = SPEC ? FL_SPEC_XF_OFF : prog[5];
    const int xf_stride = SPEC ? FL_SPEC_XF_STRIDE : prog[6], var_stride = SPEC ? FL_SPEC_VAR_STRIDE : prog[7];
#else
    const int nxf = prog[1], has_final = prog[2], pstride = prog[3], cdf_off = prog[4];
    const int xf_off = prog[5], xf_stride = prog[6], var_stride = prog[7];
#endif
    const float *__restrict__ P = params + (size_t)ts * pstride;

    if (!BINNED) for (int i = tid; i < FL_PAL_W; i += NT) palrow[i] = palette[prow * FL_PAL_W + i];
    if (BINNED) for (uint32_t i = tid; i < SETS * CNTW; i += NT) cnt[i] = 0;
    uint32_t batch_in_slot = 0;

    const size_t wi = (size_t)slot * NT + tid;
    mwc_t rctx = {rng[wi].mul, rng[wi].state, rng[wi].carry};
    float4 pt = points[wi];
    float x = pt.x, y = pt.y, color = pt.z;

    const float color_dither = 0.49f * mwc_next_11(rctx);
    if (!isfinite(fabsf(x) + fabsf(y))) reseed(x, y, color, rctx);
    __syncthreads();
    const float cam0 = P[0], cam1 = P[1], cam3 = P[3], cam4 = P[4];
    float cam2 = P[2], cam5 = P[5];
#ifdef FL_RTC
    if constexpr (SPEC && FL_HOIST_BUDGET >= 2) asm volatile("" : "+v"(cam2), "+v"(cam5));
#endif
    const float *__restrict__ xf_final = P + xf_off + nxf * xf_stride;
#ifdef FL_RTC
    constexpr bool OPAC = SPEC ? kAnyOpac : true;
#else
    constexpr bool OPAC = true;
#endif
    bool any_opac = false;
    if constexpr (OPAC && SPEC) any_opac = true;
    else if constexpr (OPAC) for (int i = 0; i < nxf; ++i) any_opac |= (__float_as_int(P[xf_off + i * xf_stride + 14]) & 0x200) != 0;
    uint32_t hid_bits = 0u;

    const float cdf_lane = ((int)l < nxf - 1 && l < 63u) ? P[cdf_off + (int)l] : -1.0f;
    auto sel_ok = [&](uint32_t s) -> bool { return (float)s * (1.0f / 4294967296.0f) <= cdf_lane; };
    const bool thr_valid = sel_ok(0u);
    uint32_t thr = 0xffffffffu;
    if (!sel_ok(thr)) {
        uint32_t lo = 0u, hi = 0xffffffffu;
        for (int it = 0; it < 32; ++it) {
            const uint32_t mid = lo + ((hi - lo) >> 1);
            if (sel_ok(mid)) lo = mid; else hi = mid;
        }
        thr = lo;
    }
    auto swap_dest = [&](const uint32_t phase) -> uint32_t {
        return pair ? (w & ~3u) * 64u + shuffle_dest<4>(w & 3u, l, phase) : shuffle_dest<NW>(w, l, phase);
    };
    uint32_t rot0 = swap_dest(round0 % 3u), rot1 = swap_dest((round0 + 1u) % 3u), rot2 = swap_dest((round0 + 2u) % 3u);
    uint32_t n_acc = 0, n_oob = 0, n_drop = 0, n_spill = 0;
    bool pend_ok = false; uint32_t pend_gi = 0; float pend_mult = 1.0f; u64 pend_old = 0;

    const unsigned long long valid_lanes = __ballot(thr_valid);
    auto choose = [&](uint32_t sel) -> int {
        const unsigned long long le = (__ballot(sel <= thr) & valid_lanes) | (1ull << 63);
        return min((int)__builtin_ctzll(le), nxf - 1);
    };
    uint32_t sel_next = __builtin_amdgcn_readfirstlane(mwc_next(rctx));
    int k_next = choose(sel_next);
    const float *__restrict__ xf_next = P + xf_off + k_next * xf_stride;
#ifdef FL_RTC
    constexpr bool RESIDENT = SPEC && kSpecResident;
    XfHead heads[FL_SPEC_NXF];
    XfVec hv[FL_SPEC_NXF] = {};
    XfTail tails[FL_SPEC_NXF] = {};
    if constexpr (RESIDENT) {
#pragma unroll
        for (int i = 0; i < FL_SPEC_NXF; ++i) {
            heads[i] = load_head(P + xf_off + i * xf_stride);
#pragma unroll
            for (int k = 0; k < kTailWords; ++k) tails[i].w[k] = (P + xf_off + i * xf_stride)[kTailFirst + k];
            if constexpr (kHoistCol) {
                const float csp = heads[i].f[13];
                hv[i].cprod = heads[i].f[12] * csp;
                asm volatile("" : "+v"(hv[i].cprod));
                heads[i].f[13] = __int_as_float(__builtin_amdgcn_readfirstlane(__float_as_int(1.0f - csp)));
            }
            if constexpr (kHoistAff) { hv[i].xo = heads[i].f[2]; hv[i].yo = heads[i].f[5]; asm volatile("" : "+v"(hv[i].xo), "+v"(hv[i].yo)); }
            if constexpr (kHoistPost) { hv[i].pxo = heads[i].f[8]; hv[i].pyo = heads[i].f[11]; asm volatile("" : "+v"(hv[i].pxo), "+v"(hv[i].pyo)); }
        }
    }
    XfHead hfin_res = {};
    XfTail tfin = {};
    XfVec vfin = {};
    if constexpr (SPEC && kHoistFinal) {
        hfin_res = load_head(xf_final);
#pragma unroll
        for (int k = 0; k < kTailWords; ++k) tfin.w[k] = xf_final[kTailFirst + k];
        const float csp = hfin_res.f[13];
        vfin.cprod = hfin_res.f[12] * csp;
        vfin.xo = hfin_res.f[2]; vfin.yo = hfin_res.f[5];
        asm volatile("" : "+v"(vfin.cprod), "+v"(vfin.xo), "+v"(vfin.yo));
        hfin_res.f[13] = __int_as_float(__builtin_amdgcn_readfirstlane(__float_as_int(1.0f - csp)));
        if constexpr (kSpecPost[FL_SPEC_NXF] != 0) { vfin.pxo = hfin_res.f[8]; vfin.pyo = hfin_res.f[11]; asm volatile("" : "+v"(vfin.pxo), "+v"(vfin.pyo)); }
    }
#else
    constexpr bool RESIDENT = false;
#endif
    XfHead hnext = RESIDENT ? XfHead{} : load_head(xf_next);
#ifdef FL_RTC
    XfTail tail_next = {};
    if constexpr (SPEC && kTab) {
#pragma unroll
        for (int i = 0; i < kTailWords; ++i) tail_next.w[i] = xf_next[kTailFirst + i];
    }
#endif
    float4 tcur = make_float4(0.0f, 0.0f, 0.0f, 0.0f);
#ifdef FL_RTC
    if constexpr (SPEC && kTab) {
        const uint32_t th = pair ? tid & 255u : tid;
        if ((int)th < FL_SPEC_NXF) {
            const float *__restrict__ rr = P + xf_off + (int)th * xf_stride;
            const float csp = rr[13];
            xtab[half * 16u + th] = make_float4(rr[2], rr[5], 1.0f - csp, rr[12] * csp);
        }
        __syncthreads();
        tcur = xtab[half * 16u + k_next];
    }
#endif

    uint32_t par = 0;
    auto advance = [&](const uint32_t dst, auto &&extra) __attribute__((always_inline)) {
        __builtin_amdgcn_s_setprio(2);
        if (!isfinite(fabsf(x) + fabsf(y))) reseed(x, y, color, rctx);

        const int k_cur = k_next;
        const float *__restrict__ xf_cur = xf_next;
#ifdef FL_RTC
        XfTail tail = tail_next;
#endif
        sel_next = __builtin_amdgcn_readfirstlane(mwc_next(rctx));
        k_next = choose(sel_next);
        xf_next = P + xf_off + k_next * xf_stride;
#ifdef FL_RTC
        if constexpr (RESIDENT) spec_dispatch_res<0, FL_SPEC_NXF>(k_cur, heads, hv, P + xf_off, xf_stride, x, y, color, rctx, tails, extra);
        else if constexpr (SPEC && kTab) spec_dispatch_tab<0, FL_SPEC_NXF>(k_cur, hnext, tcur, xf_cur, x, y, color, rctx, &tail, extra);
        else if constexpr (SPEC) spec_dispatch<0, FL_SPEC_NXF>(k_cur, hnext, xf_cur, x, y, color, rctx, extra);
        else
#endif
        { extra(); apply_xf(hnext, xf_cur, var_stride, x, y, color, rctx, any_opac); }
        if constexpr (!RESIDENT) hnext = load_head(xf_next);
#ifdef FL_RTC
        if constexpr (SPEC && kTab) {
#pragma unroll
            for (int i = 0; i < kTailWords; ++i) tail_next.w[i] = xf_next[kTailFirst + i];
        }
#endif
        (void)k_cur; (void)xf_cur;

        {
            swp[par][0][dst] = x; swp[par][1][dst] = y; swp[par][2][dst] = color;
            __syncthreads();
            x = swp[par][0][tid]; y = swp[par][1][tid]; color = swp[par][2][tid];
            if constexpr (OPAC) if (any_opac) { hid_bits = __float_as_uint(color); color = fabsf(color); }
#ifdef FL_RTC
            if constexpr (SPEC && kTab) tcur = xtab[half * 16u + k_next];
#endif
            __builtin_amdgcn_s_setprio(0);
            par ^= 1u;
        }
    };
    const uint32_t nfuse = min(fuse, nrounds);
#ifdef FL_RTC
    constexpr bool SPLIT_FUSE = !SPEC || FL_SPEC_NXF <= 9;
#else
    constexpr bool SPLIT_FUSE = true;
#endif
    constexpr bool ROT3 = SPLIT_FUSE;
    uint32_t ph = 0;
    auto next_dst = [&]() __attribute__((always_inline)) -> uint32_t {
        const uint32_t dst = rot0;
        rot0 = rot1; rot1 = rot2; rot2 = dst;
        return dst;
    };
    auto rounds = [&](uint32_t from, uint32_t to, auto body) __attribute__((always_inline)) {
        if constexpr (ROT3) {
            uint32_t i = from;
            while (i < to) {
                if (ph == 0u) { body(rot0, i); ph = 1u; if (++i == to) break; }
                if (ph == 1u) { body(rot1, i); ph = 2u; if (++i == to) break; }
                body(rot2, i); ph = 0u; ++i;
            }
        } else {
            for (uint32_t i = from; i < to; ++i) body(next_dst(), i);
        }
    };
#ifdef FL_RTC
    constexpr bool MERGE = BINNED && SPEC && SPLIT_FUSE && FL_SPEC_NXF <= FL_ITER_MERGE_MAX_XF;
#else
    constexpr bool MERGE = false;
#endif
    auto plot_head = [&](float &cx, float &cy, float &cf) __attribute__((always_inline)) {
        float fx = x, fy = y, fc = color;
#ifdef FL_RTC
        if constexpr (SPEC) {
            if constexpr (kHoistFinal) spec_apply_xf_res<FL_SPEC_NXF, true, true, true>(hfin_res, vfin, xf_final, fx, fy, fc, rctx, &tfin);
            else if constexpr (FL_SPEC_FINAL != 0) { const XfHead hfin = load_head(xf_final); spec_apply_xf<FL_SPEC_NXF>(hfin, xf_final, fx, fy, fc, rctx); }
        } else
#endif
        if (has_final) { const XfHead hfin = load_head(xf_final); apply_xf(hfin, xf_final, var_stride, fx, fy, fc, rctx); }
        cx = fmaf(cam0, fx, fmaf(cam1, fy, cam2));
        cy = fmaf(cam3, fx, fmaf(cam4, fy, cam5));
        cf = fminf(fmaxf(fmaf(fc, 255.0f, color_dither), 0.0f), 255.0f) + 8388608.0f;
        if constexpr (OPAC) if (any_opac) cf = __uint_as_float((__float_as_uint(cf) & 0x7fffffffu) | (hid_bits & 0x80000000u));
        if constexpr (MERGE) asm volatile("" : "+v"(cx), "+v"(cy), "+v"(cf));
    };
    auto plot_rest = [&](const float cx, const float cy, const float cf, const uint32_t staged) __attribute__((always_inline)) {
        const uint32_t ix = __float_as_uint(cx + 12582912.0f) - 0x4b400000u;
        const uint32_t iy = __float_as_uint(cy + 12582912.0f) - 0x4b400000u;
        bool ok = (ix < astride) & (iy < aheight);
        if constexpr (OPAC) {
            if (any_opac) {
                const bool hidden = (__float_as_uint(cf) >> 31) != 0u;
                if (COUNT) { n_drop += hidden; n_oob += !hidden & !ok; }
                ok &= !hidden;
            } else if (COUNT) n_oob += !ok;
        } else
        if (COUNT) n_oob += !ok;
        const uint32_t gi = ok ? iy * astride + ix : 0u;

        float mult = 1.0f;
        if (ok && !BINNED) {
            const uint32_t flag = (hot[gi >> 4] >> ((gi & 15u) << 1)) & 3u;
            if (flag) {
                mult = hot_mult(flag);
                if (mwc_next_01(rctx) > frcp(mult)) { ok = false; if (COUNT) ++n_drop; }
            }
        }
        const uint32_t cbits = __float_as_uint(cf);
        const int ci = (int)((cbits - 0x4b000000u) & 0xffu);
        const u64 val = BINNED ? 0ull : palrow[ci];

        if (ACC == 0) {
            drain_if_full(pend_ok, pend_old, pend_gi, pend_mult, atom, out4, n_spill);
            pend_ok = ok; pend_gi = gi; pend_mult = mult;
            if (ok) pend_old = __hip_atomic_fetch_add(atom + gi, val, __ATOMIC_RELAXED, __HIP_MEMORY_SCOPE_AGENT);
        } else if (BINNED) {
            const uint32_t bin = ok ? __umul24(iy >> FL_TILE_H_LOG2, bg.tiles_x) + (ix >> TWL) : bg.nbins;
            const uint32_t t1 = ((iy & (FL_TILE_H - 1u)) << TWL) | (ix & ((1u << TWL) - 1u));
            const uint32_t t2 = WIDE ? t1 : (bin << (TWL + FL_TILE_H_LOG2)) | t1;
            const uint32_t rec = __builtin_amdgcn_perm(t2, cbits, 0x06050400u);
            if (WIDE) skey[staged * NT + tid] = (uint16_t)bin;
            stage[staged * NT + tid] = rec;
            if constexpr (OPAC) { if (!any_opac || ok) __hip_atomic_fetch_add(my_cnt + bin, 1u, __ATOMIC_RELAXED, __HIP_MEMORY_SCOPE_WORKGROUP); }
            else __hip_atomic_fetch_add(my_cnt + bin, 1u, __ATOMIC_RELAXED, __HIP_MEMORY_SCOPE_WORKGROUP);
        } else {
            pend_old += ok ? val + gi : 0ull;
        }
        if (COUNT) n_acc += ok;
    };
    auto no_extra = []() __attribute__((always_inline)) {};
    if (SPLIT_FUSE) rounds(0u, MERGE && nfuse < nrounds ? nfuse + 1u : nfuse, [&](uint32_t dst, uint32_t) __attribute__((always_inline)) { advance(dst, no_extra); });
    uint32_t fuse_left = SPLIT_FUSE ? 0u : nfuse;
    for (uint32_t rd = SPLIT_FUSE ? nfuse : 0u; rd < nrounds;) {
    const uint32_t blen = fuse_left ? fuse_left : BINNED ? min(bg.rounds, nrounds - rd) : nrounds - rd;
    const bool plotting = fuse_left == 0u;
    fuse_left = 0u;
    if constexpr (MERGE) {
        const uint32_t last = rd + blen >= nrounds ? 1u : 0u;
        rounds(0u, blen - last, [&](const uint32_t dst, const uint32_t staged) __attribute__((always_inline)) {
            float fx, fy, fc;
            plot_head(fx, fy, fc);
            advance(dst, [&]() __attribute__((always_inline)) { plot_rest(fx, fy, fc, staged); });
        });
        if (last) { float fx, fy, fc; plot_head(fx, fy, fc); plot_rest(fx, fy, fc, blen - 1u); }
    } else
    rounds(0u, blen, [&](const uint32_t dst, const uint32_t staged) __attribute__((always_inline)) {
        advance(dst, no_extra);
        if (!SPLIT_FUSE && !plotting) return;
        float fx, fy, fc;
        plot_head(fx, fy, fc);
        plot_rest(fx, fy, fc, staged);
    });
    rd += blen;
    if (BINNED && plotting) {
            auto sort_batch = [&](const uint32_t staged) __attribute__((always_inline)) {
#if FL_SORT_LOCAL_TID
                uint32_t tid_local = threadIdx.x;
                asm volatile("" : "+v"(tid_local));
                const uint32_t tid = tid_local, l = tid & 63u;
                const uint32_t w = (uint32_t)__builtin_amdgcn_readfirstlane((int)(tid >> 6));
#endif
                const uint32_t batch_id = slot * (bg.nbatch_total / gridDim.x) + batch_in_slot;
                __syncthreads();
                uint32_t r2[FL_BIN_R_MAX], k2[FL_BIN_R_MAX];
                auto has_record = [&](const uint32_t k) __attribute__((always_inline)) -> bool {
                    if constexpr (OPAC) { if (any_opac && k == bg.nbins) return false; }
                    return k != 0xffffffffu;
                };
#pragma unroll
                for (int q = 0; q < FL_BIN_R_MAX; ++q) {
                    const bool have = (uint32_t)q < staged;
                    r2[q] = have ? stage[q * NT + tid] : 0u;
                    k2[q] = !have ? 0xffffffffu : WIDE ? (uint32_t)skey[q * NT + tid] : r2[q] >> PAY_BITS;
                }
                const uint32_t nchunk = (bg.nbins + 64u) >> 6;
                if (nchunk <= 8u) {
                    if (w == 0) {
                        uint32_t running = 0;
                        for (uint32_t c0 = 0; c0 <= bg.nbins; c0 += 64) {
                            const uint32_t b = c0 + l;
                            uint32_t vs[SETS], v = 0;
#pragma unroll
                            for (int t = 0; t < SETS; ++t) { vs[t] = b <= bg.nbins ? cnt[t * CNTW + b] : 0u; v += vs[t]; }
                            const uint32_t incl = wave_incl_scan(v, l);
                            const uint32_t excl = incl - v + running;
                            if (b <= bg.nbins) {
                                uint32_t at = excl;
#pragma unroll
                                for (int t = 0; t < SETS; ++t) { cnt[t * CNTW + b] = at; at += vs[t]; }
                            }
                            if (b < bg.nbins) bin_dir[(size_t)b * bg.nbatch_total + batch_id] = (excl << 16) | v;
                            if (b == bg.nbins) *s_nvalid = excl;
                            running += (uint32_t)__builtin_amdgcn_readlane((int)incl, 63);
                        }
                    }
                } else {
                for (uint32_t c = w; c < nchunk; c += NW) {
                    const uint32_t b = c * 64u + l;
                    uint32_t v = 0;
#pragma unroll
                    for (int t = 0; t < SETS; ++t) v += b <= bg.nbins ? cnt[t * CNTW + b] : 0u;
                    const uint32_t incl = wave_incl_scan(v, l);
                    if (l == 63u) tot[c] = incl;
                }
                __syncthreads();
                {
                    const uint32_t t0 = l < nchunk ? tot[l] : 0u, t1 = 64u + l < nchunk ? tot[64u + l] : 0u;
                    const uint32_t i0 = wave_incl_scan(t0, l);
                    const uint32_t i1 = wave_incl_scan(t1, l) + (uint32_t)__builtin_amdgcn_readlane((int)i0, 63);
                    for (uint32_t cv = w; cv < nchunk; cv += NW) {
                        const uint32_t c = (uint32_t)__builtin_amdgcn_readfirstlane((int)cv);
                        const uint32_t base = c < 64u ? (uint32_t)__builtin_amdgcn_readlane((int)(i0 - t0), c)
                                                      : (uint32_t)__builtin_amdgcn_readlane((int)(i1 - t1), c - 64u);
                        const uint32_t b = c * 64u + l;
                        uint32_t vs[SETS], v = 0;
#pragma unroll
                        for (int t = 0; t < SETS; ++t) { vs[t] = b <= bg.nbins ? cnt[t * CNTW + b] : 0u; v += vs[t]; }
                        const uint32_t excl = wave_incl_scan(v, l) - v + base;
                        if (b <= bg.nbins) {
                            uint32_t at = excl;
#pragma unroll
                            for (int t = 0; t < SETS; ++t) { cnt[t * CNTW + b] = at; at += vs[t]; }
                            if (b < bg.nbins) bin_dir[(size_t)b * bg.nbatch_total + batch_id] = (excl << 16) | v;
                            else *s_nvalid = excl;
                        }
                    }
                }
                }
                __syncthreads();
#pragma unroll
                for (int q0 = 0; q0 < FL_BIN_R_MAX; q0 += FL_SCATTER_DEPTH) {
                    if ((uint32_t)q0 >= staged) break;
                    uint32_t pos[FL_SCATTER_DEPTH];
#pragma unroll
                    for (int q = 0; q < FL_SCATTER_DEPTH; ++q)
                        if (has_record(k2[q0 + q]))
                            pos[q] = __hip_atomic_fetch_add(my_cnt + k2[q0 + q], 1u, __ATOMIC_RELAXED, __HIP_MEMORY_SCOPE_WORKGROUP);
#pragma unroll
                    for (int q = 0; q < FL_SCATTER_DEPTH; ++q)
                        if (has_record(k2[q0 + q])) stage[pos[q]] = r2[q0 + q] & ((1u << PAY_BITS) - 1u);
                }
                __syncthreads();
                const uint32_t nvalid = *s_nvalid;
                if constexpr (PACK3) {
                    typedef uint32_t u32x2_ __attribute__((ext_vector_type(2)));
                    u32x2_ *d2 = reinterpret_cast<u32x2_ *>(bin_log) + (size_t)batch_id * fl_pack3_words(bg.rounds * NT);
                    const uint32_t nwords = (nvalid + 2u) / 3u;
                    for (uint32_t i = tid; i < nwords; i += NT) {
                        const uint32_t a = stage[3u * i], b = stage[3u * i + 1u], c3 = stage[3u * i + 2u];
                        u32x2_ o;
                        o.x = a | (b << 21); o.y = (b >> 11) | (c3 << 10);
                        __builtin_nontemporal_store(o, d2 + i);
                    }
                } else {
                uint4 *dst = reinterpret_cast<uint4 *>(bin_log + (size_t)batch_id * bg.rounds * NT);
                {
                    typedef uint32_t u32x4_ __attribute__((ext_vector_type(4)));
                    const u32x4_ *s4 = reinterpret_cast<const u32x4_ *>(stage);
                    u32x4_ *d4 = reinterpret_cast<u32x4_ *>(dst);
                    for (uint32_t i = tid; i * 4 < nvalid; i += NT) __builtin_nontemporal_store(s4[i], d4 + i);
                }
                }
                for (uint32_t i = tid; i < SETS * CNTW; i += NT) cnt[i] = 0;
                ++batch_in_slot;
                __syncthreads();
            };
#if FL_SORT_FULL_COPY
            if (blen == (uint32_t)FL_BIN_R_MAX) sort_batch((uint32_t)FL_BIN_R_MAX); else
#endif
            sort_batch(blen);
    }
    }

    if (ACC == 0) drain_if_full(pend_ok, pend_old, pend_gi, pend_mult, atom, out4, n_spill);
    else if (pend_old == 0x123456789abcdefull) atom[0] = pend_old;
    {
        uint32_t tid_end = threadIdx.x;
        asm volatile("" : "+v"(tid_end));
        const size_t wj = (size_t)slot * NT + tid_end;
        points[wj] = make_float4(x, y, color, 0.0f);
        rng[wj].mul = rctx.mul; rng[wj].state = rctx.state; rng[wj].carry = rctx.carry;
    }

    if (COUNT) {
        atomicAdd(counters + 0, (u64)n_acc);
        atomicAdd(counters + 1, (u64)n_oob);
        atomicAdd(counters + 2, (u64)n_drop);
        atomicAdd(counters + 3, (u64)n_spill);
    }
}

#define FL_ITER_ARGS const int32_t *__restrict__ prog, const float *__restrict__ params, \
       const u64 *__restrict__ palette, fl_mwc *__restrict__ rng, float4 *__restrict__ points, \
       const uint32_t *__restrict__ hot, u64 *__restrict__ atom, float *__restrict__ out4, \
       u64 *__restrict__ counters, uint32_t astride, uint32_t aheight, \
       uint32_t round0, uint32_t nrounds, uint32_t fuse, BinGeom bg, \
       uint32_t *__restrict__ bin_log, uint32_t *__restrict__ bin_dir
#define FL_ITER_PASS prog, params, palette, rng, points, hot, atom, out4, counters, astride, aheight, round0, nrounds, fuse, bg, bin_log, bin_dir

#ifdef FL_RTC
extern "C" __global__ void __launch_bounds__(FL_SPEC_NW * 64) k_iter_spec(FL_ITER_ARGS)
{
    extern __shared__ __attribute__((aligned(16))) unsigned char smem[];
    iter_body<FL_SPEC_NW, FL_SPEC_COUNT != 0, FL_SPEC_ACC, true>(smem, FL_ITER_PASS);
}
#else
template <int NW, bool COUNT, int ACC>
__global__ void __launch_bounds__(NW * 64, NW == 4 ? 6 : NW == 8 ? 3 : 1) k_iter(FL_ITER_ARGS)
{
    extern __shared__ __attribute__((aligned(16))) unsigned char smem[];
    iter_body<NW, COUNT, ACC, false>(smem, FL_ITER_PASS);
}

__global__ void __launch_bounds__(256)
k_apply_xf_tap(const int32_t *__restrict__ prog, const float *__restrict__ params, uint32_t ts, int xfi,
               uint32_t n, float4 *__restrict__ pts, fl_mwc *__restrict__ rng)
{
    const uint32_t i = blockIdx.x * 256u + threadIdx.x;
    if (i >= n) return;
    const float *__restrict__ P = params + (size_t)ts * prog[3];
    mwc_t r = {rng[i].mul, rng[i].state, rng[i].carry};
    float4 p = pts[i];
    const float *__restrict__ xf = P + prog[5] + xfi * prog[6];
    const XfHead h = load_head(xf);
    apply_xf(h, xf, prog[7], p.x, p.y, p.z, r);
    pts[i] = p;
    rng[i].mul = r.mul; rng[i].state = r.state; rng[i].carry = r.carry;
}

void launch_apply_xf_tap(hipStream_t st, const int32_t *prog, const float *params, uint32_t ts, int xfi,
                         uint32_t n, float4 *pts, fl_mwc *rng)
{
    hipLaunchKernelGGL(k_apply_xf_tap, dim3((n + 255) / 256), dim3(256), 0, st, prog, params, ts, xfi, n, pts, rng);
}

template <int NW>
__global__ void __launch_bounds__(NW * 64) k_shuffle_tap(uint32_t *out, uint32_t round)
{
    __shared__ uint32_t s[NW * 64];
    const uint32_t tid = threadIdx.x;
    s[shuffle_dest<NW>(tid >> 6, tid & 63, round % 3u)] = tid;
    __syncthreads();
    out[tid] = s[tid];
}

__global__ void __launch_bounds__(256)
k_flush(u64 *__restrict__ atom, float4 *__restrict__ out, uint32_t *__restrict__ hot, uint32_t nbins, int use_hot)
{
    const uint32_t gi = blockIdx.x * 256u + threadIdx.x;
    if (gi >= nbins) return;
    const uint32_t sh = (gi & 15u) << 1;
    const uint32_t flag = use_hot ? (hot[gi >> 4] >> sh) & 3u : 0u;
    const float mult = hot_mult(flag);
    const u64 cell = __builtin_nontemporal_load(atom + gi);
    __builtin_nontemporal_store(0ull, atom + gi);
    float yf, uf, vf, df;
    unpack_cell(cell, yf, uf, vf, df);
    float4 o = out[gi];
    const float m255 = mult * FL_INV255;
    o.w = fmaf(df, mult, o.w);
    o.x = fmaf(yf, m255, o.x);
    o.y = fmaf(uf, m255, o.y);
    o.z = fmaf(vf, m255, o.z);
    out[gi] = o;
    uint32_t nf = (uint32_t)(o.w > 128.0f) + (uint32_t)(o.w > 512.0f) + (uint32_t)(o.w > 2048.0f);
    uint32_t word = nf << sh;
    word |= __shfl_xor(word, 1);
    word |= __shfl_xor(word, 2);
    word |= __shfl_xor(word, 4);
    word |= __shfl_xor(word, 8);
    if ((gi & 15u) == 0) hot[gi >> 4] = word;
}

static size_t iter_lds_bytes(int nw, int acc, uint32_t rounds, uint32_t nbins, uint32_t sub_log2)
{
    size_t nt = (size_t)nw * 64, b = 2 * 3 * nt * 4;
    if (acc == 1 || acc == 3) b += (size_t)rounds * nt * (acc == 3 ? 6 : 4) + (nw == 4 ? FL_CNT_SETS : FL_CNT_SETS_BIG) * (size_t)((nbins + 1 + 3) & ~3u) * 4 + 16
             + 128 * 4;
    else b += FL_PAL_W * 8;
    return b + ((size_t)FL_XTAB_BYTES << sub_log2);
}

void launch_iter(hipStream_t st, int nw, bool count, int acc, uint32_t nslots,
                 const int32_t *prog, const float *params, const u64 *palette, fl_mwc *rng,
                 float4 *points, const uint32_t *hot, u64 *atom, float *out4, u64 *counters,
                 uint32_t astride, uint32_t aheight, uint32_t round0, uint32_t nrounds, uint32_t fuse,
                 uint32_t tiles_x, uint32_t nbins, uint32_t rounds_per_batch, uint32_t nbatch_total,
                 uint32_t *log, uint32_t *dir, hipEvent_t ev_start, hipEvent_t ev_stop, uint32_t sub_log2)
{
    if (sub_log2 != 0u && (4 << sub_log2) != nw) abort();
    BinGeom bg = {tiles_x, nbins, rounds_per_batch, nbatch_total, sub_log2};
    const size_t lds = iter_lds_bytes(nw, acc, rounds_per_batch, nbins, sub_log2);
#define LAUNCH(NW, C, A) do { \
        static unsigned long long attr_done = 0; \
        ensure_max_dynamic_lds((const void *)k_iter<NW, C, A>, attr_done); \
         \
        hipExtLaunchKernelGGL((k_iter<NW, C, A>), dim3(nslots), dim3(NW * 64), lds, st, ev_start, ev_stop, 0, prog, params, palette, \
        rng, points, hot, atom, out4, counters, astride, aheight, round0, nrounds, fuse, bg, log, dir); } while (0)
#define LAUNCH_NW(C, A) do { if (nw == 4) LAUNCH(4, C, A); else if (nw == 8) LAUNCH(8, C, A); else LAUNCH(16, C, A); } while (0)
    if (acc == 2) LAUNCH_NW(false, 2);
    else if (acc == 1) { if (count) LAUNCH_NW(true, 1); else LAUNCH_NW(false, 1); }
    else if (acc == 3) { if (count) LAUNCH_NW(true, 3); else LAUNCH_NW(false, 3); }
    else { if (count) LAUNCH_NW(true, 0); else LAUNCH_NW(false, 0); }
#undef LAUNCH_NW
#undef LAUNCH
}

void launch_iter_fn(hipStream_t st, hipFunction_t fn, int nw, int acc, uint32_t nslots,
                    const int32_t *prog, const float *params, const u64 *palette, fl_mwc *rng,
                    float4 *points, const uint32_t *hot, u64 *atom, float *out4, u64 *counters,
                    uint32_t astride, uint32_t aheight, uint32_t round0, uint32_t nrounds, uint32_t fuse,
                    uint32_t tiles_x, uint32_t nbins, uint32_t rounds_per_batch, uint32_t nbatch_total,
                    uint32_t *log, uint32_t *dir, hipEvent_t ev_start, hipEvent_t ev_stop, uint32_t sub_log2)
{
    if (sub_log2 != 0u && (4 << sub_log2) != nw) abort();
    BinGeom bg = {tiles_x, nbins, rounds_per_batch, nbatch_total, sub_log2};
    const size_t lds = iter_lds_bytes(nw, acc, rounds_per_batch, nbins, sub_log2);
    void *args[] = {&prog, &params, &palette, &rng, &points, &hot, &atom, &out4, &counters, &astride, &aheight,
                    &round0, &nrounds, &fuse, &bg, &log, &dir};
    (void)hipExtModuleLaunchKernel(fn, nslots * (uint32_t)nw * 64, 1, 1, (uint32_t)nw * 64, 1, 1, lds, st, args, nullptr, ev_start, ev_stop, 0);
}

void launch_flush(hipStream_t st, u64 *atom, float4 *out, uint32_t *hot, uint32_t nbins, bool use_hot)
{
    hipLaunchKernelGGL(k_flush, dim3((nbins + 255) / 256), dim3(256), 0, st, atom, out, hot, nbins, use_hot ? 1 : 0);
}

__global__ void __launch_bounds__(256)
k_clear_frame(float4 *__restrict__ front, u64 *__restrict__ atom, uint32_t *__restrict__ hot, u64 *__restrict__ counters,
              float4 *__restrict__ points, uint32_t nbins, uint32_t npoints)
{
    const uint32_t i = blockIdx.x * 256u + threadIdx.x;
    if (i < nbins) {
        front[i] = make_float4(0.0f, 0.0f, 0.0f, 0.0f);
        atom[i] = 0ull;
        if ((i & 15u) == 0u) hot[i >> 4] = 0u;
    }
    if (i < npoints) {
        const float nanf_ = __uint_as_float(0x7fc00000u);
        points[i] = make_float4(nanf_, nanf_, nanf_, nanf_);
    }
    if (i < 4u) counters[i] = 0ull;
}

void launch_clear_frame(hipStream_t st, float4 *front, u64 *atom, uint32_t *hot, u64 *counters, float4 *points,
                        uint32_t nbins, uint32_t npoints)
{
    const uint32_t n = nbins > npoints ? nbins : npoints;
    hipLaunchKernelGGL(k_clear_frame, dim3((n + 255) / 256), dim3(256), 0, st, front, atom, hot, counters, points, nbins, npoints);
}

void launch_shuffle_tap(hipStream_t st, int nw, uint32_t *out, uint32_t round)
{
    if (nw == 4) hipLaunchKernelGGL(k_shuffle_tap<4>, dim3(1), dim3(256), 0, st, out, round);
    else if (nw == 8) hipLaunchKernelGGL(k_shuffle_tap<8>, dim3(1), dim3(512), 0, st, out, round);
    else hipLaunchKernelGGL(k_shuffle_tap<16>, dim3(1), dim3(1024), 0, st, out, round);
}
#endif
```

cuburn_amd/csrc/kernels.h:

```cpp
#pragma once
#include <hip/hip_runtime.h>
#include <stdint.h>
#include "../../include/flame_hip.h"

typedef unsigned long long u64;

static inline void ensure_max_dynamic_lds(const void *fn, unsigned long long &done)
{
    int dev = 0;
    if (hipGetDevice(&dev) != hipSuccess || dev < 0 || dev > 63) dev = 63;
    if (done >> dev & 1ull) return;
    hipFuncSetAttribute(fn, hipFuncAttributeMaxDynamicSharedMemorySize, 160 * 1024);
    if (dev != 63) done |= 1ull << dev;
}

void launch_iter(hipStream_t st, int nw, bool count, int acc, uint32_t nslots,
                 const int32_t *prog, const float *params, const u64 *palette, fl_mwc *rng,
                 float4 *points, const uint32_t *hot, u64 *atom, float *out4, u64 *counters,
                 uint32_t astride, uint32_t aheight, uint32_t round0, uint32_t nrounds, uint32_t fuse,
                 uint32_t tiles_x, uint32_t nbins, uint32_t rounds_per_batch, uint32_t nbatch_total,
                 uint32_t *log, uint32_t *dir,
                 hipEvent_t ev_start = nullptr, hipEvent_t ev_stop = nullptr, uint32_t sub_log2 = 0);
void launch_flush(hipStream_t st, u64 *atom, float4 *out, uint32_t *hot, uint32_t nbins, bool use_hot);
void launch_clear_frame(hipStream_t st, float4 *front, u64 *atom, uint32_t *hot, u64 *counters, float4 *points,
                        uint32_t nbins, uint32_t npoints);
void launch_shuffle_tap(hipStream_t st, int nw, uint32_t *out, uint32_t round);
void launch_apply_xf_tap(hipStream_t st, const int32_t *prog, const float *params, uint32_t ts, int xfi,
                         uint32_t n, float4 *pts, fl_mwc *rng);

#include <string>
#include <vector>
struct IterSpec {
    int nxf = 0, has_final = 0, pstride = 0, cdf_off = 0, xf_off = 0, xf_stride = 0, var_stride = 0;
    std::vector<int> nvar, post, opac;
    std::vector<std::vector<int>> vids;
};
bool rtc_available();
unsigned rtc_epoch();
int rtc_compile(const IterSpec &spec, int nw, bool count, int acc, std::vector<char> *code, std::string *err, const char *extra_opt = nullptr, uint32_t sub_log2 = 0);
int rtc_iter_kernel(int device, const IterSpec &spec, int nw, uint32_t nslots, bool count, int acc, hipFunction_t *fn, std::string *err, uint32_t sub_log2 = 0);
void launch_iter_fn(hipStream_t st, hipFunction_t fn, int nw, int acc, uint32_t nslots,
                    const int32_t *prog, const float *params, const u64 *palette, fl_mwc *rng,
                    float4 *points, const uint32_t *hot, u64 *atom, float *out4, u64 *counters,
                    uint32_t astride, uint32_t aheight, uint32_t round0, uint32_t nrounds, uint32_t fuse,
                    uint32_t tiles_x, uint32_t nbins, uint32_t rounds_per_batch, uint32_t nbatch_total,
                    uint32_t *log, uint32_t *dir, hipEvent_t ev_start, hipEvent_t ev_stop, uint32_t sub_log2 = 0);

void launch_accum_tiles(hipStream_t st, const uint32_t *log, const uint32_t *dir, const u64 *palette,
                        u64 *atom, float *out4, uint32_t tiles_x, uint32_t nbins, uint32_t nparts,
                        uint32_t nbatch_total, uint32_t batch_records, uint32_t nslots,
                        uint32_t astride, uint32_t aheight, bool wide);

void launch_interp_palette(hipStream_t st, fl_mwc *rng_pal, const float *ptimes, const float4 *pals,
                           float ts, float tstep, u64 *out);
void launch_interp_params(hipStream_t st, float *params, const float *times, const float *knots,
                          const int32_t *ops, uint32_t nops, uint32_t pstride, uint32_t nts, float ts, float tstep,
                          fl_dim dim, bool zero_first);

void launch_yuv_to_rgb(hipStream_t st, fl_dim d, float4 *dst, const float4 *src);
void launch_den_blur_1c(hipStream_t st, fl_dim d, float *dst, const float *src, int pattern, int upsample, const float *coefs7);
void launch_full_blur(hipStream_t st, fl_dim d, float4 *dst, const float4 *src, int pattern, int upsample, const float *coefs7);
void launch_logscale(hipStream_t st, fl_dim d, float4 *buf, float k1, float k2);
void launch_colorclip(hipStream_t st, fl_dim d, float4 *buf, float vib, float highpow, float gam, float lin, float lingam);
void launch_gamma_full_hi(hipStream_t st, fl_dim d, float4 *dst, const float4 *src);
void launch_smearclip(hipStream_t st, fl_dim d, float4 *buf, const float4 *smear, float gam_m_1, float lin, float lingam);
void launch_apply_gamma(hipStream_t st, fl_dim d, float *dst, const float4 *src, float gamma);
void launch_haloclip(hipStream_t st, fl_dim d, float4 *buf, const float *den, float gam_m_1);
void launch_plainclip(hipStream_t st, fl_dim d, float4 *buf, float gam_m_1, float lin, float lingam, float brightness);
void launch_logencode(hipStream_t st, fl_dim d, float4 *dst, const float4 *src, float degamma);

struct DeTail { int do_log; float k1, k2; int do_clip; float vib, highpow, gam, lin, lingam; int order; };
void launch_de_dir(hipStream_t st, fl_dim d, int pattern, float4 *Nout, const float4 *N, const float *coefs7,
                   float sstd, float cstd, float dstd, float dpow, float gspeed, int in_mode = 1, const DeTail *tail = nullptr);

void launch_de_adaptive(hipStream_t st, fl_dim d, float4 *buf, float4 *stage_c, float *stage_a, uint32_t *tmax,
                        const float *sinv, float R, float Rmin, float curve);
size_t de_adaptive_tiles(fl_dim d);
void de_adaptive_norms(float *out);

void launch_f32_to_rgba(hipStream_t st, fl_dim d, const float4 *src, fl_mwc *rng, uint32_t nrng, int fmt, void *dst);

int launch_measure_copy(size_t nbytes, int iters, float *ms);

int launch_sort_pass(hipStream_t st, uint32_t *dst, const uint32_t *src, uint32_t n, uint32_t lo_bit, uint32_t nbits,
                     int ignore_max, uint32_t *hist, uint32_t *chunk_tot, uint32_t *total_dev);
size_t sort_scratch_words(uint32_t n, uint32_t nbits, size_t *chunk_words);
```

cuburn_amd/csrc/rtc.hip:

```cpp
#include <hip/hip_runtime.h>
#include <hip/hiprtc.h>
#include <dlfcn.h>
#include <cstdio>
#include <cstring>
#include <map>
#include <mutex>
#include <string>
#include <vector>
#include "kernels.h"
#include "flame_device.h"
#define FL_STR2(x) #x
#define FL_STR(x) FL_STR2(x)
#include "rtc_sources.inc"

namespace {

struct Api {
    bool ok = false;
    hiprtcResult (*create)(hiprtcProgram *, const char *, const char *, int, const char **, const char **) = nullptr;
    hiprtcResult (*compile)(hiprtcProgram, int, const char **) = nullptr;
    hiprtcResult (*log_size)(hiprtcProgram, size_t *) = nullptr;
    hiprtcResult (*log)(hiprtcProgram, char *) = nullptr;
    hiprtcResult (*code_size)(hiprtcProgram, size_t *) = nullptr;
    hiprtcResult (*code)(hiprtcProgram, char *) = nullptr;
    hiprtcResult (*destroy)(hiprtcProgram *) = nullptr;
};

Api load_api()
{
    Api a;
    void *h = nullptr;
    for (const char *name : {"libhiprtc.so.7", "libhiprtc.so", "/opt/rocm/lib/libhiprtc.so"}) {
        h = dlopen(name, RTLD_NOW | RTLD_LOCAL);
        if (h) break;
    }
    if (!h) return a;
#define SYM(field, sym) a.field = reinterpret_cast<decltype(a.field)>(dlsym(h, sym)); if (!a.field) return a
    SYM(create, "hiprtcCreateProgram"); SYM(compile, "hiprtcCompileProgram");
    SYM(log_size, "hiprtcGetProgramLogSize"); SYM(log, "hiprtcGetProgramLog");
    SYM(code_size, "hiprtcGetCodeSize"); SYM(code, "hiprtcGetCode"); SYM(destroy, "hiprtcDestroyProgram");
#undef SYM
    a.ok = true;
    return a;
}

const Api &api() { static Api a = load_api(); return a; }

struct Entry { hipModule_t mod = nullptr; hipFunction_t fn = nullptr; };
std::mutex g_mu;
std::map<std::string, Entry> g_cache;
unsigned g_epoch = 1;
const size_t kMaxModules = 64;

std::string spec_header(const IterSpec &s, int nw, bool count, int acc, uint32_t sub_log2)
{
    const int nrec = s.nxf + s.has_final;
    int maxv = 1;
    for (int i = 0; i < nrec; ++i) maxv = std::max(maxv, s.nvar[i]);
    std::string h = "// generated: structure of one genome (rtc.hip)\n";
    char buf[256];
#define DEF(name, val) snprintf(buf, sizeof buf, "#define %s %d\n", name, (int)(val)); h += buf
    DEF("FL_SPEC_NXF", s.nxf); DEF("FL_SPEC_FINAL", s.has_final); DEF("FL_SPEC_PSTRIDE", s.pstride);
    DEF("FL_SPEC_CDF_OFF", s.cdf_off); DEF("FL_SPEC_XF_OFF", s.xf_off); DEF("FL_SPEC_XF_STRIDE", s.xf_stride);
    DEF("FL_SPEC_VAR_STRIDE", s.var_stride); DEF("FL_SPEC_NW", nw); DEF("FL_SPEC_COUNT", count ? 1 : 0); DEF("FL_SPEC_ACC", acc);
    DEF("FL_SPEC_SUB_LOG2", sub_log2 != 0u && (4 << sub_log2) == nw ? (int)sub_log2 : 0);
#undef DEF
    h += "constexpr int kSpecNvar[] = {";
    for (int i = 0; i < nrec; ++i) h += std::to_string(s.nvar[i]) + ",";
    h += "0};\nconstexpr int kSpecPost[] = {";
    for (int i = 0; i < nrec; ++i) h += std::to_string(s.post[i]) + ",";
    h += "0};\nconstexpr int kSpecOpac[] = {";
    for (int i = 0; i < nrec; ++i) h += std::to_string(i < (int)s.opac.size() ? s.opac[i] : 0) + ",";
    snprintf(buf, sizeof buf, "0};\nconstexpr int kSpecVid[][%d] = {", maxv);
    h += buf;
    for (int i = 0; i < nrec; ++i) {
        h += "{";
        for (int j = 0; j < maxv; ++j) h += std::to_string(j < s.nvar[i] ? s.vids[i][j] : 0) + ",";
        h += "},";
    }
    h += "{0}};\n";
    return h;
}

}

bool rtc_available() { return api().ok; }

int rtc_compile(const IterSpec &spec, int nw, bool count, int acc, std::vector<char> *code, std::string *err, const char *extra_opt, uint32_t sub_log2)
{
    const Api &a = api();
    if (!a.ok) { *err = "libhiprtc not found"; return -1; }
    const std::string header = spec_header(spec, nw, count, acc, sub_log2);
    hiprtcProgram prog = nullptr;
    const char *hdr_src[] = {rtc_src_variations, rtc_src_device, rtc_src_abi, header.c_str()};
    const char *hdr_name[] = {"variations.h", "flame_device.h", "flame_hip.h", "flame_spec.h"};
    if (a.create(&prog, rtc_src_iter, "iter.hip", 4, hdr_src, hdr_name) != HIPRTC_SUCCESS) { *err = "hiprtcCreateProgram failed"; return -1; }
    std::string arch_opt = "--offload-arch=gfx950";
    {
        int dev = 0;
        hipDeviceProp_t prop;
        if (hipGetDevice(&dev) == hipSuccess && hipGetDeviceProperties(&prop, dev) == hipSuccess && prop.gcnArchName[0]) {
            std::string name(prop.gcnArchName);
            arch_opt = "--offload-arch=" + name.substr(0, name.find(':'));
        } else (void)hipGetLastError();
    }
    const char *opts[] = {arch_opt.c_str(), "-O3", "-std=c++20", "-ffp-contract=off", "-DFL_RTC=1",
                          "-mllvm", "-structurizecfg-skip-uniform-regions=true",
                          "-DFL_LOG_PACK3=" FL_STR(FL_LOG_PACK3),
                          "-fno-slp-vectorize",
    };
    std::vector<const char *> optv(opts, opts + sizeof opts / sizeof *opts);
    if (extra_opt) optv.push_back(extra_opt);
    std::vector<std::string> extra;
    if (const char *e = getenv("FLAME_RTC_FLAGS")) {
        std::string w;
        for (const char *q = e;; ++q) {
            if (*q && *q != ' ') { w += *q; continue; }
            if (!w.empty()) { extra.push_back(w); w.clear(); }
            if (!*q) break;
        }
        for (const std::string &x : extra) optv.push_back(x.c_str());
    }
    const hiprtcResult rc = a.compile(prog, (int)optv.size(), optv.data());
    if (rc != HIPRTC_SUCCESS) {
        size_t n = 0;
        a.log_size(prog, &n);
        std::string log(n, '\0');
        if (n) a.log(prog, &log[0]);
        *err = "hiprtc compile failed: " + log.substr(0, 4000);
        a.destroy(&prog);
        return -1;
    }
    size_t n = 0;
    a.code_size(prog, &n);
    code->resize(n);
    a.code(prog, code->data());
    a.destroy(&prog);
    if (const char *dir = getenv("FLAME_RTC_DUMP")) {
        const std::string d(dir);
        if (FILE *f = fopen((d + "/flame_spec.h").c_str(), "w")) { fwrite(header.data(), 1, header.size(), f); fclose(f); }
        if (FILE *f = fopen((d + "/k_iter_spec.co").c_str(), "wb")) { fwrite(code->data(), 1, code->size(), f); fclose(f); }
    }
    return 0;
}

unsigned rtc_epoch() { std::lock_guard<std::mutex> lock(g_mu); return g_epoch; }

int rtc_iter_kernel(int device, const IterSpec &spec, int nw, uint32_t nslots, bool count, int acc, hipFunction_t *fn, std::string *err, uint32_t sub_log2)
{
    const uint32_t wps = (nslots * 4u + 1023u) / 1024u;
    const int reg_limit = nw == 4 && wps >= 1u && wps <= 8u ? (int)(512u / wps / 8u * 8u) : 0;
    const std::string key = std::to_string(device) + "|" + std::to_string(reg_limit) + "|" + spec_header(spec, nw, count, acc, sub_log2);
    std::lock_guard<std::mutex> lock(g_mu);
    auto it = g_cache.find(key);
    if (it != g_cache.end()) { *fn = it->second.fn; return 0; }
    Entry e;
    const char *budgets[] = {nullptr, "-DFL_HOIST_BUDGET=7", "-DFL_HOIST_BUDGET=5", "-DFL_HOIST_BUDGET=0"};
    Entry first; bool have_first = false;
    for (int b = 0; b < 4; ++b) {
        std::vector<char> code;
        if (rtc_compile(spec, nw, count, acc, &code, err, budgets[b], sub_log2)) { if (have_first) break; return -1; }
        Entry t;
        if (hipModuleLoadData(&t.mod, code.data()) != hipSuccess) { (void)hipGetLastError(); *err = "hipModuleLoadData failed"; if (have_first) break; return -1; }
        if (hipModuleGetFunction(&t.fn, t.mod, "k_iter_spec") != hipSuccess) {
            (void)hipGetLastError(); (void)hipModuleUnload(t.mod); *err = "k_iter_spec not found in the compiled module"; if (have_first) break; return -1;
        }
        int regs = 0;
        if (hipFuncGetAttribute(&regs, HIP_FUNC_ATTRIBUTE_NUM_REGS, t.fn) != hipSuccess) { (void)hipGetLastError(); regs = 0; }
        if (reg_limit == 0 || regs <= reg_limit) { if (have_first) (void)hipModuleUnload(first.mod); have_first = false; e = t; break; }
        if (!have_first) { first = t; have_first = true; } else (void)hipModuleUnload(t.mod);
    }
    if (have_first) e = first;
    err->clear();
    if (g_cache.size() >= kMaxModules) {
        (void)hipDeviceSynchronize();
        const std::string prefix = std::to_string(device) + "|";
        for (auto kv = g_cache.begin(); kv != g_cache.end();) {
            if (kv->first.compare(0, prefix.size(), prefix) == 0) { (void)hipModuleUnload(kv->second.mod); kv = g_cache.erase(kv); }
            else ++kv;
        }
        ++g_epoch;
    }
    g_cache[key] = e;
    *fn = e.fn;
    return 0;
}
```

include/flame_hip.h:

```cpp
#ifndef FLAME_HIP_H
#define FLAME_HIP_H

#ifndef __HIPCC_RTC__
#include <stdint.h>
#include <stddef.h>
#endif

#ifdef __cplusplus
extern "C" {
#endif

#define FL_ABI_VERSION 1

enum {
    FL_OK = 0,
    FL_E_INVAL = -1,
    FL_E_NOMEM = -2,
    FL_E_HIP = -3,
    FL_E_NODEV = -4,
    FL_E_UNSUPPORTED = -5
};

typedef struct fl_dim {
    uint32_t w, h, aw, ah, astride;
} fl_dim;

typedef struct fl_mwc {
    uint32_t mul, state, carry;
} fl_mwc;

#define FL_KNOTS 32
#define FL_NTEMPORAL 1024
#define FL_PAL_W 256
#define FL_PAL_H 64
#define FL_GUTTER 12

#define FL_PROG_MAGIC 0x464c5032
#define FL_PROG_HDR 8
#define FL_MAX_XFORMS 64
#define FL_MAX_PSTRIDE 4096
#define FL_XF_HDR 16

enum {
    FL_OP_SPLINE = 0,
    FL_OP_SPLINE_MAG = 1,
    FL_OP_CAMERA = 2,
    FL_OP_AFFINE = 3,
    FL_OP_CDF = 4,
    FL_OP_RATIO2 = 5,
    FL_OP_INVSQ = 6,
    FL_OP_PERSP = 7,
    FL_OP_INVSQ_MAX = 8,
    FL_OP_CONST = 9,
    FL_OP_OPACITY = 10
};


typedef struct fl_ctx fl_ctx;
typedef struct fl_genome fl_genome;

int fl_abi_version(void);
const char *fl_last_error(void);

void fl_calc_dim(uint32_t w, uint32_t h, fl_dim *out);

int fl_ctx_create(int device, void *stream, const fl_mwc *seeds, uint32_t nseeds, uint32_t nslots, fl_ctx **out);
void fl_ctx_destroy(fl_ctx *ctx);
int fl_ctx_sync(fl_ctx *ctx);

int fl_genome_create(fl_ctx *ctx, const int32_t *prog, uint32_t nprog,
                     const int32_t *ops, uint32_t nops, uint32_t nrows, fl_genome **out);
void fl_genome_destroy(fl_genome *g);

int fl_genome_upload(fl_ctx *ctx, fl_genome *g, const float *times, const float *knots,
                     const float *pal_rgba, const float *pal_times, uint32_t npal);

int fl_interp(fl_ctx *ctx, fl_genome *g, uint32_t w, uint32_t h, float ts, float td);

enum {
    FL_ACCUM_ATOMIC = 0,
    FL_ACCUM_BINNED = 1
};

int fl_iterate(fl_ctx *ctx, fl_genome *g, uint32_t w, uint32_t h, double nsamples,
               uint32_t fuse, int accum_mode, uint64_t *nsamples_run);

enum {
    FL_FILT_YUV = 0,
    FL_FILT_BILATERAL = 1,
    FL_FILT_LOGSCALE = 2,
    FL_FILT_COLORCLIP = 3,
    FL_FILT_SMEARCLIP = 4,
    FL_FILT_HALOCLIP = 5,
    FL_FILT_PLAINCLIP = 6,
    FL_FILT_LOGENCODE = 7,
    FL_FILT_DE = 8
};
#define FL_DE_MAX_RADIUS 96
int fl_filter(fl_ctx *ctx, int filter_id, uint32_t w, uint32_t h, const float *params, uint32_t nparams);

enum {
    FL_OUT_RGBA8 = 0,
    FL_OUT_RGBA16 = 1,
    FL_OUT_YUV444P = 2,
    FL_OUT_YUV444P10 = 3,
    FL_OUT_YUV420P10 = 4,
    FL_OUT_YUV444P12 = 5
};
size_t fl_output_bytes(uint32_t w, uint32_t h, int fmt);
int fl_output(fl_ctx *ctx, uint32_t w, uint32_t h, int fmt, void *host_out, uint64_t dev_out);

int fl_sort_u32(fl_ctx *ctx, uint64_t dst_dev, uint64_t src_dev, uint32_t n, uint32_t lo_bit, uint32_t nbits, int ignore_max,
                uint32_t *nvalid);

int fl_frame_begin(fl_ctx *ctx, uint32_t *frame_id);
int fl_frame_ms(fl_ctx *ctx, uint32_t frame_id, float *ms);
int fl_frame_query(fl_ctx *ctx, uint32_t frame_id);

void *fl_host_alloc(size_t nbytes);
void fl_host_free(void *p);

int fl_timings_reset(fl_ctx *ctx);
int fl_timings(fl_ctx *ctx, float *iter_ms, float *flush_ms, float *filter_ms, uint32_t *niter_launches);
int fl_timings_detail(fl_ctx *ctx, float ms[6]);
int fl_launch_stats(fl_ctx *ctx, uint32_t out[4]);
int fl_measure_copy(int device, size_t nbytes, int iters, float *ms);

enum {
    FL_BUF_FRONT = 0,
    FL_BUF_BACK = 1,
    FL_BUF_PARAMS = 2,
    FL_BUF_PALETTE = 3,
    FL_BUF_POINTS = 4,
    FL_BUF_SEEDS = 5,
    FL_BUF_ATOM = 6,
    FL_BUF_HOT = 7,
    FL_BUF_SIDE = 8
};
int fl_read_buffer(fl_ctx *ctx, fl_genome *g, int which, void *host_dst, size_t nbytes);
int fl_write_buffer(fl_ctx *ctx, fl_genome *g, int which, const void *host_src, size_t nbytes);

int fl_buffer_ptr(fl_ctx *ctx, fl_genome *g, int which, void **dev_ptr, size_t *nbytes);
int fl_buffer_ptr_async(fl_ctx *ctx, fl_genome *g, int which, void **dev_ptr, size_t *nbytes);
int fl_stream_dependency(fl_ctx *ctx, void *stream, int ctx_waits);
int fl_reserve(fl_ctx *ctx, uint32_t w, uint32_t h);

int fl_debug_iter_launch(fl_ctx *ctx, fl_genome *g, uint32_t w, uint32_t h, uint32_t round0,
                         uint32_t nrounds, uint32_t fuse, int accum_mode);
int fl_debug_flush(fl_ctx *ctx, uint32_t w, uint32_t h);
int fl_debug_clear(fl_ctx *ctx, uint32_t w, uint32_t h, int reset_points);
int fl_debug_clear_hot(fl_ctx *ctx, uint32_t w, uint32_t h);
int fl_debug_shuffle(fl_ctx *ctx, uint32_t round, uint32_t *out256);
int fl_debug_apply_xf(fl_ctx *ctx, fl_genome *g, uint32_t ts, int xfi, uint32_t n, float *xyzw, fl_mwc *rng);
int fl_rtc_compile_check(const int32_t *prog, uint32_t nprog, const int32_t *ops, uint32_t nops, int nw, int count, int acc,
                         char *log, size_t log_bytes);
int fl_debug_counters(fl_ctx *ctx, uint64_t out4[4]);


#ifdef __cplusplus
}
#endif
#endif
```

Measured before the change: 216,400 Msamples/s.

## Bake frame geometry constants into per-genome RTC iterate kernels

Extends the runtime-compiled per-genome iterate kernel so frame geometry (stride, height, tile counts, bins, rounds, slots, batches per slot) becomes compile-time constants. The compiler can then strength-reduce bin index math (shift for power-of-two tile counts), fully unroll the bin prefix-scan over a known chunk count, and use 32-bit directory indexing. A two-entry per-genome geometry cache and a per-family LRU of compiled modules limit recompiles, but a geometry change still costs a compile, and evicting a module forces a device sync.

Result: no change. 217,400 Msamples/s, median of 2 (+0.5%).

```diff
diff --git a/cuburn_amd/_lib.py b/cuburn_amd/_lib.py
--- a/cuburn_amd/_lib.py
+++ b/cuburn_amd/_lib.py
@@ -61,6 +61,8 @@
     'fl_debug_shuffle': (C.c_int, [C.c_void_p, C.c_uint32, C.c_void_p]),
     'fl_debug_counters': (C.c_int, [C.c_void_p, C.c_void_p]),
     'fl_rtc_compile_check': (C.c_int, [C.c_void_p, C.c_uint32, C.c_void_p, C.c_uint32, C.c_int, C.c_int, C.c_int, C.c_char_p, C.c_size_t]),
+    'fl_rtc_compile_check_geom': (C.c_int, [C.c_void_p, C.c_uint32, C.c_void_p, C.c_uint32, C.c_int, C.c_int, C.c_int, C.c_uint32, C.c_uint32,
+                                           C.c_uint32, C.c_uint32, C.c_char_p, C.c_size_t, C.c_char_p, C.c_size_t]),
     'fl_debug_apply_xf': (C.c_int, [C.c_void_p, C.c_void_p, C.c_uint32, C.c_int, C.c_uint32, C.c_void_p, C.c_void_p]),
 }
 EXPORTS = sorted(_SIGS)
diff --git a/cuburn_amd/csrc/flame_abi.hip b/cuburn_amd/csrc/flame_abi.hip
--- a/cuburn_amd/csrc/flame_abi.hip
+++ b/cuburn_amd/csrc/flame_abi.hip
@@ -90,11 +90,13 @@
 #define OTHER(c) ((c)->lanes[((c)->cur + (c)->nlanes - 1) % (c)->nlanes])
 #define FL_NOUT 65536u
 
+struct RtcFn { hipFunction_t fn = nullptr; SpecGeom want, baked; };
+
 struct fl_genome {
     uint64_t serial = 0;
     std::vector<int32_t> prog;
     IterSpec spec;
-    hipFunction_t rtc_fn[5][2][4] = {};
+    RtcFn rtc_fn[5][2][4][2] = {};
     unsigned rtc_epoch = 0;
     bool rtc_failed = false;
     uint32_t nops = 0, nrows = 0, pstride = 0;
@@ -540,15 +542,20 @@
 #define FL_BIN_MAX_ROUNDS 1024u
 #define FL_BIN_MAX_ROUNDS_LONG 2304u
 
-static int ensure_binned(fl_ctx *c, const fl_dim &d, uint32_t write_rounds, int buf, uint32_t *tiles_x, uint32_t *nbins,
-                         uint32_t *nbatch_total, bool *wide)
-{
-    const uint32_t nt = (uint32_t)c->nw * 64;
+static void bin_tiles(const fl_dim &d, bool force_wide, uint32_t *tiles_x, uint32_t *nbins, bool *wide)
+{
     const uint32_t rows = (d.ah + FL_TILE_H - 1) / FL_TILE_H;
-    *wide = ((d.astride + 127) / 128) * rows > FL_MAX_BINS || c->env_bin_wide;
+    *wide = ((d.astride + 127) / 128) * rows > FL_MAX_BINS || force_wide;
     const uint32_t tw = *wide ? (1u << FL_TILE_W_WIDE_LOG2) : 128u;
     *tiles_x = (d.astride + tw - 1) / tw;
     *nbins = *tiles_x * rows;
+}
+
+static int ensure_binned(fl_ctx *c, const fl_dim &d, uint32_t write_rounds, int buf, uint32_t *tiles_x, uint32_t *nbins,
+                         uint32_t *nbatch_total, bool *wide)
+{
+    const uint32_t nt = (uint32_t)c->nw * 64;
+    bin_tiles(d, c->env_bin_wide, tiles_x, nbins, wide);
     if (*nbins > FL_MAX_BINS_WIDE) return fail(FL_E_UNSUPPORTED, "image too large for the binned accumulate (> 8191 tiles of 256x64)", __FILE__, __LINE__);
     const uint32_t per_slot = (write_rounds + c->bin_rounds - 1) / c->bin_rounds;
     *nbatch_total = per_slot * c->nslots;
@@ -570,7 +577,7 @@
 }
 
 static int do_iter_launch(fl_ctx *c, fl_genome *g, const fl_dim &d, uint32_t nrounds, uint32_t fuse, bool count, int acc = 0,
-                          int buf = 0, hipStream_t drain = nullptr)
+                          int buf = 0, hipStream_t drain = nullptr, bool steady = true)
 {
     if (!drain) drain = L(c).stream;
     uint32_t tiles_x = 0, nbins = 0, nbatch_total = 0;
@@ -583,26 +590,36 @@
     EvPair *e = ev_pair(c, c->iter_ev);
     const int kacc = acc == FL_ACCUM_BINNED && wide ? 3 : acc;
     hipFunction_t fn = nullptr;
+    SpecGeom baked;
     if (c->use_rtc && !g->rtc_failed && kacc != 2) {
         const unsigned ep = rtc_epoch();
-        if (g->rtc_epoch != ep) { memset(g->rtc_fn, 0, sizeof g->rtc_fn); g->rtc_epoch = ep; }
-        hipFunction_t &slot = g->rtc_fn[c->sub_log2 ? 2 + c->sub_log2 : c->nw == 16 ? 2 : c->nw == 8][count ? 1 : 0][kacc];
-        if (!slot) {
+        if (g->rtc_epoch != ep) { for (auto &a : g->rtc_fn) for (auto &b : a) for (auto &k : b) for (auto &s : k) s = RtcFn(); g->rtc_epoch = ep; }
+        RtcFn (&slot)[2] = g->rtc_fn[c->sub_log2 ? 2 + c->sub_log2 : c->nw == 16 ? 2 : c->nw == 8][count ? 1 : 0][kacc];
+        SpecGeom want;
+        want.astride = d.astride; want.aheight = d.ah; want.tiles_x = tiles_x; want.nbins = nbins;
+        want.rounds = acc == FL_ACCUM_BINNED ? c->bin_rounds : 0u; want.nslots = c->nslots;
+        want.nbatch_slot = steady ? nbatch_total / c->nslots : 0u;
+        if (slot[1].fn && slot[1].want == want) std::swap(slot[0], slot[1]);
+        if (!slot[0].fn || !(slot[0].want == want)) {
             std::string err;
-            if (rtc_iter_kernel(c->device, g->spec, c->nw, c->nslots, count, kacc, &slot, &err, c->sub_log2)) {
+            slot[1] = slot[0];
+            slot[0] = RtcFn();
+            if (rtc_iter_kernel(c->device, g->spec, c->nw, c->nslots, count, kacc, &slot[0].fn, &err, c->sub_log2, &want, &slot[0].baked)) {
                 g->rtc_failed = true;
-                slot = nullptr;
+                slot[0].fn = nullptr;
                 fprintf(stderr, "libflame_hip: per-genome kernel not available (%s); using the interpreter kernel\n", err.c_str());
             }
+            slot[0].want = want;
         }
-        fn = slot;
+        fn = slot[0].fn;
+        baked = slot[0].baked;
     }
     (fn ? c->n_spec_launch : c->n_interp_launch) += 1;
     if (fn)
         launch_iter_fn(L(c).stream, fn, c->nw, kacc, c->nslots, g->d_prog, L(c).d_params, L(c).d_palette, c->d_rng, c->d_points,
                        L(c).d_hot, L(c).d_atom, (float *)L(c).d_front, c->d_counters, d.astride, d.ah, c->round_counter, nrounds, fuse,
                        tiles_x, nbins, c->bin_rounds, nbatch_total, L(c).d_log[buf], L(c).d_dir[buf],
-                       e ? e->a : nullptr, e ? e->b : nullptr, c->sub_log2);
+                       e ? e->a : nullptr, e ? e->b : nullptr, c->sub_log2, &baked);
     else
     launch_iter(L(c).stream, c->nw, count, kacc, c->nslots, g->d_prog, L(c).d_params, L(c).d_palette, c->d_rng, c->d_points,
                 L(c).d_hot, L(c).d_atom, (float *)L(c).d_front, c->d_counters, d.astride, d.ah, c->round_counter, nrounds, fuse,
@@ -686,7 +703,7 @@
         const uint32_t f = k == 0 ? fuse : 0;
         const int buf = pipelined ? (int)(k & 1u) : 0;
         if (pipelined && k >= 2) HIPCHK(hipStreamWaitEvent(L(c).stream, L(c).ev_ac[buf], 0));
-        if ((rc = do_iter_launch(c, g, d, (uint32_t)n + f, f, false, accum_mode, buf, drain))) return rc;
+        if ((rc = do_iter_launch(c, g, d, (uint32_t)n + f, f, false, accum_mode, buf, drain, n == std::min(batch * unit, cap)))) return rc;
         if ((rc = do_flush(c, d, accum_mode != FL_ACCUM_BINNED, drain))) return rc;
         if (pipelined) HIPCHK(hipEventRecord(L(c).ev_ac[buf], drain));
         rounds -= n;
@@ -1137,8 +1154,8 @@
     return FL_OK;
 }
 
-int fl_rtc_compile_check(const int32_t *prog, uint32_t nprog, const int32_t *ops, uint32_t nops, int nw, int count, int acc,
-                         char *log, size_t log_bytes)
+static int compile_check(const int32_t *prog, uint32_t nprog, const int32_t *ops, uint32_t nops, int nw, int count, int acc,
+                         char *log, size_t log_bytes, const SpecGeom *geom, char *key, size_t key_bytes)
 {
     REQUIRE(prog && ops && nprog >= FL_PROG_HDR && (nw == 4 || nw == 8 || nw == 16) && acc >= 0 && acc <= 3, "bad argument");
     int rc = check_prog(prog, nprog);
@@ -1165,12 +1182,44 @@
     }
     std::vector<char> code;
     std::string err;
-    rc = rtc_compile(spec, nw, (count & 1) != 0, acc, &code, &err, nullptr, (count & 2) == 0 ? 0u : nw == 8 ? 1u : nw == 16 ? 2u : 0u);
+    const uint32_t sub_log2 = (count & 2) == 0 ? 0u : nw == 8 ? 1u : nw == 16 ? 2u : 0u;
+    if (key && key_bytes) {
+        const std::string k = rtc_key(spec, nw, (count & 1) != 0, acc, sub_log2, geom);
+        uint64_t h = 1469598103934665603ull;
+        for (const unsigned char ch : k) { h ^= ch; h *= 1099511628211ull; }
+        snprintf(key, key_bytes, "%016llx", (unsigned long long)h);
+    }
+    rc = rtc_compile(spec, nw, (count & 1) != 0, acc, &code, &err, nullptr, sub_log2, geom);
     if (log && log_bytes) { snprintf(log, log_bytes, "%s", rc ? err.c_str() : "ok"); }
     if (rc) return fail(rtc_available() ? FL_E_HIP : FL_E_UNSUPPORTED, "per-genome kernel did not compile", __FILE__, __LINE__);
     return (int)(code.size() > 0 ? FL_OK : FL_E_HIP);
 }
 
+int fl_rtc_compile_check(const int32_t *prog, uint32_t nprog, const int32_t *ops, uint32_t nops, int nw, int count, int acc,
+                         char *log, size_t log_bytes)
+{
+    return compile_check(prog, nprog, ops, nops, nw, count, acc, log, log_bytes, nullptr, nullptr, 0);
+}
+
+int fl_rtc_compile_check_geom(const int32_t *prog, uint32_t nprog, const int32_t *ops, uint32_t nops, int nw, int count, int acc,
+                              uint32_t w, uint32_t h, uint32_t nslots, uint32_t write_rounds, char *log, size_t log_bytes,
+                              char *key, size_t key_bytes)
+{
+    REQUIRE(w && h && nslots && (acc == 0 || write_rounds), "bad frame geometry");
+    fl_dim d; fl_calc_dim(w, h, &d);
+    SpecGeom geom;
+    geom.astride = d.astride; geom.aheight = d.ah; geom.nslots = nslots;
+    if (acc == 1 || acc == 3) {
+        bool wide = false;
+        bin_tiles(d, acc == 3, &geom.tiles_x, &geom.nbins, &wide);
+        REQUIRE(wide == (acc == 3), "acc does not match the frame: 1 is for frames of up to FL_MAX_BINS tiles of 128x64, 3 for larger ones");
+        geom.rounds = 16;
+        if (const char *e = getenv("FLAME_BIN_ROUNDS")) { int v = atoi(e); if (v >= 1 && v <= FL_BIN_R_MAX) geom.rounds = (uint32_t)v; }
+        geom.nbatch_slot = (write_rounds + geom.rounds - 1) / geom.rounds;
+    }
+    return compile_check(prog, nprog, ops, nops, nw, count, acc, log, log_bytes, &geom, key, key_bytes);
+}
+
 int fl_debug_counters(fl_ctx *c, uint64_t out4[4])
 {
     REQUIRE(c && out4, "null argument");
diff --git a/cuburn_amd/csrc/iter.hip b/cuburn_amd/csrc/iter.hip
--- a/cuburn_amd/csrc/iter.hip
+++ b/cuburn_amd/csrc/iter.hip
@@ -72,6 +72,26 @@
 
 #ifdef FL_RTC
 #include "flame_spec.h"
+
+#ifndef FL_SPEC_GEOM
+#define FL_SPEC_GEOM 0
+#endif
+#if !FL_SPEC_GEOM
+#undef FL_SPEC_ASTRIDE
+#undef FL_SPEC_AHEIGHT
+#undef FL_SPEC_TILES_X
+#undef FL_SPEC_NBINS
+#undef FL_SPEC_ROUNDS
+#undef FL_SPEC_NSLOTS
+#undef FL_SPEC_NBATCH_SLOT
+#define FL_SPEC_ASTRIDE 0
+#define FL_SPEC_AHEIGHT 0
+#define FL_SPEC_TILES_X 0
+#define FL_SPEC_NBINS 0
+#define FL_SPEC_ROUNDS 0
+#define FL_SPEC_NSLOTS 0
+#define FL_SPEC_NBATCH_SLOT 0
+#endif
 
 constexpr int kTailFirst = FL_XF_HDR + 2, kTailWords = 10;
 struct XfTail { float w[kTailWords]; };
@@ -257,11 +277,25 @@
 iter_body(unsigned char *smem, const int32_t *__restrict__ prog, const float *__restrict__ params,
           const u64 *__restrict__ palette, fl_mwc *__restrict__ rng, float4 *__restrict__ points,
           const uint32_t *__restrict__ hot, u64 *__restrict__ atom, float *__restrict__ out4,
-          u64 *__restrict__ counters, uint32_t astride, uint32_t aheight,
-          uint32_t round0, uint32_t nrounds, uint32_t fuse, BinGeom bg,
+          u64 *__restrict__ counters, const uint32_t astride_arg, const uint32_t aheight_arg,
+          uint32_t round0, uint32_t nrounds, uint32_t fuse, const BinGeom bg_arg,
           uint32_t *__restrict__ bin_log, uint32_t *__restrict__ bin_dir)
 {
     constexpr int NT = NW * 64;
+#ifdef FL_RTC
+    constexpr bool GEOM = SPEC && FL_SPEC_GEOM != 0;
+    constexpr uint32_t kNslots = GEOM ? FL_SPEC_NSLOTS : 0u, kBatchSlot = GEOM ? FL_SPEC_NBATCH_SLOT : 0u;
+    constexpr uint32_t kTilesX = GEOM ? FL_SPEC_TILES_X : 0u, kNbins = GEOM ? FL_SPEC_NBINS : 0u;
+    const uint32_t astride = GEOM ? (uint32_t)FL_SPEC_ASTRIDE : astride_arg, aheight = GEOM ? (uint32_t)FL_SPEC_AHEIGHT : aheight_arg;
+    const BinGeom bg = GEOM ? BinGeom{FL_SPEC_TILES_X, FL_SPEC_NBINS, FL_SPEC_ROUNDS, kBatchSlot ? kBatchSlot * kNslots : bg_arg.nbatch_total, bg_arg.sub_log2}
+                            : bg_arg;
+#else
+    constexpr bool GEOM = false;
+    constexpr uint32_t kNslots = 0u, kBatchSlot = 0u, kTilesX = 0u, kNbins = 0u;
+    const uint32_t astride = astride_arg, aheight = aheight_arg;
+    const BinGeom bg = bg_arg;
+#endif
+    const uint32_t nslots = kNslots ? kNslots : gridDim.x;
     constexpr int SETS = NW == 4 ? FL_CNT_SETS : FL_CNT_SETS_BIG;
     constexpr bool BINNED = ACC == 1 || ACC == 3, WIDE = ACC == 3;
     constexpr bool PACK3 = FL_LOG_PACK3 != 0 && ACC == 1;
@@ -287,7 +321,7 @@
     const uint32_t sub_log2 = NW == 4 ? 0u : SPEC ? kSubSpec : bg.sub_log2;
     const bool pair = sub_log2 != 0u;
     const uint32_t half = pair ? (uint32_t)__builtin_amdgcn_readfirstlane((int)(w >> 2)) : 0u;
-    const uint32_t slot = blockIdx.x, ts = pair ? (slot << sub_log2) + half : slot, prow = slot * FL_PAL_H / gridDim.x;
+    const uint32_t slot = blockIdx.x, ts = pair ? (slot << sub_log2) + half : slot, prow = slot * FL_PAL_H / nslots;
 #ifdef FL_RTC
     const int nxf = SPEC ? FL_SPEC_NXF : prog[1], has_final = SPEC ? FL_SPEC_FINAL : prog[2], pstride = SPEC ? FL_SPEC_PSTRIDE : prog[3];
     const int cdf_off = SPEC ? FL_SPEC_CDF_OFF : prog[4], xf_off = SPEC ? FL_SPEC_XF_OFF : prog[5];
@@ -530,7 +564,9 @@
             pend_ok = ok; pend_gi = gi; pend_mult = mult;
             if (ok) pend_old = __hip_atomic_fetch_add(atom + gi, val, __ATOMIC_RELAXED, __HIP_MEMORY_SCOPE_AGENT);
         } else if (BINNED) {
-            const uint32_t bin = ok ? __umul24(iy >> FL_TILE_H_LOG2, bg.tiles_x) + (ix >> TWL) : bg.nbins;
+            constexpr bool TX_POW2 = GEOM && kTilesX != 0 && (kTilesX & (kTilesX - 1)) == 0;
+            const uint32_t trow = iy >> FL_TILE_H_LOG2;
+            const uint32_t bin = ok ? (TX_POW2 ? trow << (uint32_t)__builtin_ctz(kTilesX | 0x80000000u) : __umul24(trow, bg.tiles_x)) + (ix >> TWL) : bg.nbins;
             const uint32_t t1 = ((iy & (FL_TILE_H - 1u)) << TWL) | (ix & ((1u << TWL) - 1u));
             const uint32_t t2 = WIDE ? t1 : (bin << (TWL + FL_TILE_H_LOG2)) | t1;
             const uint32_t rec = __builtin_amdgcn_perm(t2, cbits, 0x06050400u);
@@ -575,7 +611,7 @@
                 const uint32_t tid = tid_local, l = tid & 63u;
                 const uint32_t w = (uint32_t)__builtin_amdgcn_readfirstlane((int)(tid >> 6));
 #endif
-                const uint32_t batch_id = slot * (bg.nbatch_total / gridDim.x) + batch_in_slot;
+                const uint32_t batch_id = slot * (kBatchSlot ? kBatchSlot : bg.nbatch_total / nslots) + batch_in_slot;
                 __syncthreads();
                 uint32_t r2[FL_BIN_R_MAX], k2[FL_BIN_R_MAX];
                 auto has_record = [&](const uint32_t k) __attribute__((always_inline)) -> bool {
@@ -589,6 +625,41 @@
                     k2[q] = !have ? 0xffffffffu : WIDE ? (uint32_t)skey[q * NT + tid] : r2[q] >> PAY_BITS;
                 }
                 const uint32_t nchunk = (bg.nbins + 64u) >> 6;
+                constexpr bool DIR32 = GEOM && kBatchSlot != 0u && (u64)kNbins * kBatchSlot * kNslots < (1ull << 30);
+                auto dir_at = [&](const uint32_t b) __attribute__((always_inline)) -> uint32_t * {
+                    if constexpr (DIR32) return bin_dir + (b * bg.nbatch_total + batch_id);
+                    else return bin_dir + ((size_t)b * bg.nbatch_total + batch_id);
+                };
+                constexpr uint32_t kChunks = GEOM ? (kNbins + 64u) >> 6 : 0u;
+                if constexpr (GEOM && kChunks <= 8u) {
+                    if (w == 0) {
+                        constexpr uint32_t NB = kNbins;
+                        constexpr uint32_t NC = kChunks ? kChunks : 1u;
+                        uint32_t vs[NC][SETS], v[NC];
+#pragma unroll
+                        for (uint32_t c = 0; c < kChunks; ++c) {
+                            const uint32_t b = c * 64u + l;
+                            v[c] = 0;
+#pragma unroll
+                            for (int t = 0; t < SETS; ++t) { vs[c][t] = (c * 64u + 63u <= NB || b <= NB) ? cnt[t * CNTW + b] : 0u; v[c] += vs[c][t]; }
+                        }
+                        uint32_t running = 0;
+#pragma unroll
+                        for (uint32_t c = 0; c < kChunks; ++c) {
+                            const uint32_t b = c * 64u + l;
+                            const uint32_t incl = wave_incl_scan(v[c], l);
+                            const uint32_t excl = incl - v[c] + running;
+                            if (c * 64u + 63u <= NB || b <= NB) {
+                                uint32_t at = excl;
+#pragma unroll
+                                for (int t = 0; t < SETS; ++t) { cnt[t * CNTW + b] = at; at += vs[c][t]; }
+                            }
+                            if (c * 64u + 63u < NB || b < NB) *dir_at(b) = (excl << 16) | v[c];
+                            if (c == kChunks - 1u && b == NB) *s_nvalid = excl;
+                            if (c + 1u < kChunks) running += (uint32_t)__builtin_amdgcn_readlane((int)incl, 63);
+                        }
+                    }
+                } else
                 if (nchunk <= 8u) {
                     if (w == 0) {
                         uint32_t running = 0;
@@ -604,7 +675,7 @@
 #pragma unroll
                                 for (int t = 0; t < SETS; ++t) { cnt[t * CNTW + b] = at; at += vs[t]; }
                             }
-                            if (b < bg.nbins) bin_dir[(size_t)b * bg.nbatch_total + batch_id] = (excl << 16) | v;
+                            if (b < bg.nbins) *dir_at(b) = (excl << 16) | v;
                             if (b == bg.nbins) *s_nvalid = excl;
                             running += (uint32_t)__builtin_amdgcn_readlane((int)incl, 63);
                         }
@@ -636,7 +707,7 @@
                             uint32_t at = excl;
 #pragma unroll
                             for (int t = 0; t < SETS; ++t) { cnt[t * CNTW + b] = at; at += vs[t]; }
-                            if (b < bg.nbins) bin_dir[(size_t)b * bg.nbatch_total + batch_id] = (excl << 16) | v;
+                            if (b < bg.nbins) *dir_at(b) = (excl << 16) | v;
                             else *s_nvalid = excl;
                         }
                     }
@@ -826,9 +897,16 @@
                     float4 *points, const uint32_t *hot, u64 *atom, float *out4, u64 *counters,
                     uint32_t astride, uint32_t aheight, uint32_t round0, uint32_t nrounds, uint32_t fuse,
                     uint32_t tiles_x, uint32_t nbins, uint32_t rounds_per_batch, uint32_t nbatch_total,
-                    uint32_t *log, uint32_t *dir, hipEvent_t ev_start, hipEvent_t ev_stop, uint32_t sub_log2)
+                    uint32_t *log, uint32_t *dir, hipEvent_t ev_start, hipEvent_t ev_stop, uint32_t sub_log2, const SpecGeom *baked)
 {
     if (sub_log2 != 0u && (4 << sub_log2) != nw) abort();
+    if (baked && baked->astride != 0u &&
+        (baked->astride != astride || baked->aheight != aheight || baked->tiles_x != tiles_x || baked->nbins != nbins ||
+         baked->rounds != ((acc == 1 || acc == 3) ? rounds_per_batch : 0u) || baked->nslots != nslots ||
+         (baked->nbatch_slot != 0u && (u64)baked->nbatch_slot * nslots != nbatch_total))) {
+        fprintf(stderr, "libflame_hip: per-genome kernel launched with a frame geometry it was not compiled for\n");
+        abort();
+    }
     BinGeom bg = {tiles_x, nbins, rounds_per_batch, nbatch_total, sub_log2};
     const size_t lds = iter_lds_bytes(nw, acc, rounds_per_batch, nbins, sub_log2);
     void *args[] = {&prog, &params, &palette, &rng, &points, &hot, &atom, &out4, &counters, &astride, &aheight,
diff --git a/cuburn_amd/csrc/kernels.h b/cuburn_amd/csrc/kernels.h
--- a/cuburn_amd/csrc/kernels.h
+++ b/cuburn_amd/csrc/kernels.h
@@ -35,16 +35,27 @@
     std::vector<int> nvar, post, opac;
     std::vector<std::vector<int>> vids;
 };
+struct SpecGeom {
+    uint32_t astride = 0, aheight = 0, tiles_x = 0, nbins = 0, rounds = 0, nslots = 0, nbatch_slot = 0;
+    bool operator==(const SpecGeom &o) const {
+        return astride == o.astride && aheight == o.aheight && tiles_x == o.tiles_x && nbins == o.nbins && rounds == o.rounds &&
+               nslots == o.nslots && nbatch_slot == o.nbatch_slot;
+    }
+};
 bool rtc_available();
 unsigned rtc_epoch();
-int rtc_compile(const IterSpec &spec, int nw, bool count, int acc, std::vector<char> *code, std::string *err, const char *extra_opt = nullptr, uint32_t sub_log2 = 0);
-int rtc_iter_kernel(int device, const IterSpec &spec, int nw, uint32_t nslots, bool count, int acc, hipFunction_t *fn, std::string *err, uint32_t sub_log2 = 0);
+int rtc_compile(const IterSpec &spec, int nw, bool count, int acc, std::vector<char> *code, std::string *err, const char *extra_opt = nullptr, uint32_t sub_log2 = 0,
+                const SpecGeom *geom = nullptr);
+std::string rtc_key(const IterSpec &spec, int nw, bool count, int acc, uint32_t sub_log2, const SpecGeom *geom);
+int rtc_iter_kernel(int device, const IterSpec &spec, int nw, uint32_t nslots, bool count, int acc, hipFunction_t *fn, std::string *err, uint32_t sub_log2 = 0,
+                    const SpecGeom *geom = nullptr, SpecGeom *baked = nullptr);
 void launch_iter_fn(hipStream_t st, hipFunction_t fn, int nw, int acc, uint32_t nslots,
                     const int32_t *prog, const float *params, const u64 *palette, fl_mwc *rng,
                     float4 *points, const uint32_t *hot, u64 *atom, float *out4, u64 *counters,
                     uint32_t astride, uint32_t aheight, uint32_t round0, uint32_t nrounds, uint32_t fuse,
                     uint32_t tiles_x, uint32_t nbins, uint32_t rounds_per_batch, uint32_t nbatch_total,
-                    uint32_t *log, uint32_t *dir, hipEvent_t ev_start, hipEvent_t ev_stop, uint32_t sub_log2 = 0);
+                    uint32_t *log, uint32_t *dir, hipEvent_t ev_start, hipEvent_t ev_stop, uint32_t sub_log2 = 0,
+                    const SpecGeom *baked = nullptr);
 
 void launch_accum_tiles(hipStream_t st, const uint32_t *log, const uint32_t *dir, const u64 *palette,
                         u64 *atom, float *out4, uint32_t tiles_x, uint32_t nbins, uint32_t nparts,
diff --git a/cuburn_amd/csrc/rtc.hip b/cuburn_amd/csrc/rtc.hip
--- a/cuburn_amd/csrc/rtc.hip
+++ b/cuburn_amd/csrc/rtc.hip
@@ -46,13 +46,26 @@
 
 const Api &api() { static Api a = load_api(); return a; }
 
-struct Entry { hipModule_t mod = nullptr; hipFunction_t fn = nullptr; };
+struct Entry {
+    hipModule_t mod = nullptr; hipFunction_t fn = nullptr;
+    SpecGeom geom;
+    std::string family;
+    unsigned long long seq = 0;
+};
 std::mutex g_mu;
 std::map<std::string, Entry> g_cache;
 unsigned g_epoch = 1;
 const size_t kMaxModules = 64;
-
-std::string spec_header(const IterSpec &s, int nw, bool count, int acc, uint32_t sub_log2)
+const size_t kMaxGeoms = 8;
+unsigned long long g_seq = 0;
+
+bool geom_off()
+{
+    const char *e = getenv("FLAME_RTC_FLAGS");
+    return e && strstr(e, "-DFL_SPEC_GEOM=0");
+}
+
+std::string spec_header(const IterSpec &s, int nw, bool count, int acc, uint32_t sub_log2, const SpecGeom *geom = nullptr)
 {
     const int nrec = s.nxf + s.has_final;
     int maxv = 1;
@@ -64,6 +77,12 @@
     DEF("FL_SPEC_CDF_OFF", s.cdf_off); DEF("FL_SPEC_XF_OFF", s.xf_off); DEF("FL_SPEC_XF_STRIDE", s.xf_stride);
     DEF("FL_SPEC_VAR_STRIDE", s.var_stride); DEF("FL_SPEC_NW", nw); DEF("FL_SPEC_COUNT", count ? 1 : 0); DEF("FL_SPEC_ACC", acc);
     DEF("FL_SPEC_SUB_LOG2", sub_log2 != 0u && (4 << sub_log2) == nw ? (int)sub_log2 : 0);
+    if (geom && geom->astride != 0u && !geom_off()) {
+        h += "#ifndef FL_SPEC_GEOM\n#define FL_SPEC_GEOM 1\n#endif\n";
+        DEF("FL_SPEC_ASTRIDE", geom->astride); DEF("FL_SPEC_AHEIGHT", geom->aheight); DEF("FL_SPEC_TILES_X", geom->tiles_x);
+        DEF("FL_SPEC_NBINS", geom->nbins); DEF("FL_SPEC_ROUNDS", geom->rounds); DEF("FL_SPEC_NSLOTS", geom->nslots);
+        DEF("FL_SPEC_NBATCH_SLOT", geom->nbatch_slot);
+    }
 #undef DEF
     h += "constexpr int kSpecNvar[] = {";
     for (int i = 0; i < nrec; ++i) h += std::to_string(s.nvar[i]) + ",";
@@ -86,11 +105,18 @@
 
 bool rtc_available() { return api().ok; }
 
-int rtc_compile(const IterSpec &spec, int nw, bool count, int acc, std::vector<char> *code, std::string *err, const char *extra_opt, uint32_t sub_log2)
+std::string rtc_key(const IterSpec &spec, int nw, bool count, int acc, uint32_t sub_log2, const SpecGeom *geom)
+{
+    const char *e = getenv("FLAME_RTC_FLAGS");
+    return std::string(e ? e : "") + "|" + spec_header(spec, nw, count, acc, sub_log2, geom);
+}
+
+int rtc_compile(const IterSpec &spec, int nw, bool count, int acc, std::vector<char> *code, std::string *err, const char *extra_opt, uint32_t sub_log2,
+                const SpecGeom *geom)
 {
     const Api &a = api();
     if (!a.ok) { *err = "libhiprtc not found"; return -1; }
-    const std::string header = spec_header(spec, nw, count, acc, sub_log2);
+    const std::string header = spec_header(spec, nw, count, acc, sub_log2, geom);
     hiprtcProgram prog = nullptr;
     const char *hdr_src[] = {rtc_src_variations, rtc_src_device, rtc_src_abi, header.c_str()};
     const char *hdr_name[] = {"variations.h", "flame_device.h", "flame_hip.h", "flame_spec.h"};
@@ -146,20 +172,23 @@
 
 unsigned rtc_epoch() { std::lock_guard<std::mutex> lock(g_mu); return g_epoch; }
 
-int rtc_iter_kernel(int device, const IterSpec &spec, int nw, uint32_t nslots, bool count, int acc, hipFunction_t *fn, std::string *err, uint32_t sub_log2)
-{
+int rtc_iter_kernel(int device, const IterSpec &spec, int nw, uint32_t nslots, bool count, int acc, hipFunction_t *fn, std::string *err, uint32_t sub_log2,
+                    const SpecGeom *geom, SpecGeom *baked)
+{
+    if (geom && (geom->astride == 0u || geom_off())) geom = nullptr;
     const uint32_t wps = (nslots * 4u + 1023u) / 1024u;
     const int reg_limit = nw == 4 && wps >= 1u && wps <= 8u ? (int)(512u / wps / 8u * 8u) : 0;
-    const std::string key = std::to_string(device) + "|" + std::to_string(reg_limit) + "|" + spec_header(spec, nw, count, acc, sub_log2);
+    const std::string prefix = std::to_string(device) + "|" + std::to_string(reg_limit) + "|";
+    const std::string key = prefix + rtc_key(spec, nw, count, acc, sub_log2, geom);
     std::lock_guard<std::mutex> lock(g_mu);
     auto it = g_cache.find(key);
-    if (it != g_cache.end()) { *fn = it->second.fn; return 0; }
+    if (it != g_cache.end()) { *fn = it->second.fn; if (baked) *baked = it->second.geom; return 0; }
     Entry e;
     const char *budgets[] = {nullptr, "-DFL_HOIST_BUDGET=7", "-DFL_HOIST_BUDGET=5", "-DFL_HOIST_BUDGET=0"};
     Entry first; bool have_first = false;
     for (int b = 0; b < 4; ++b) {
         std::vector<char> code;
-        if (rtc_compile(spec, nw, count, acc, &code, err, budgets[b], sub_log2)) { if (have_first) break; return -1; }
+        if (rtc_compile(spec, nw, count, acc, &code, err, budgets[b], sub_log2, geom)) { if (have_first) break; return -1; }
         Entry t;
         if (hipModuleLoadData(&t.mod, code.data()) != hipSuccess) { (void)hipGetLastError(); *err = "hipModuleLoadData failed"; if (have_first) break; return -1; }
         if (hipModuleGetFunction(&t.fn, t.mod, "k_iter_spec") != hipSuccess) {
@@ -181,7 +210,26 @@
         }
         ++g_epoch;
     }
+    if (geom) {
+        e.geom = *geom;
+        e.family = prefix + rtc_key(spec, nw, count, acc, sub_log2, nullptr);
+        size_t n = 0;
+        auto oldest = g_cache.end();
+        for (auto kv = g_cache.begin(); kv != g_cache.end(); ++kv) {
+            if (kv->second.family != e.family) continue;
+            ++n;
+            if (oldest == g_cache.end() || kv->second.seq < oldest->second.seq) oldest = kv;
+        }
+        if (n >= kMaxGeoms) {
+            (void)hipDeviceSynchronize();
+            (void)hipModuleUnload(oldest->second.mod);
+            g_cache.erase(oldest);
+            ++g_epoch;
+        }
+    }
+    e.seq = ++g_seq;
     g_cache[key] = e;
     *fn = e.fn;
+    if (baked) *baked = e.geom;
     return 0;
 }
diff --git a/include/flame_hip.h b/include/flame_hip.h
--- a/include/flame_hip.h
+++ b/include/flame_hip.h
@@ -154,6 +154,9 @@
 int fl_debug_apply_xf(fl_ctx *ctx, fl_genome *g, uint32_t ts, int xfi, uint32_t n, float *xyzw, fl_mwc *rng);
 int fl_rtc_compile_check(const int32_t *prog, uint32_t nprog, const int32_t *ops, uint32_t nops, int nw, int count, int acc,
                          char *log, size_t log_bytes);
+int fl_rtc_compile_check_geom(const int32_t *prog, uint32_t nprog, const int32_t *ops, uint32_t nops, int nw, int count, int acc,
+                              uint32_t w, uint32_t h, uint32_t nslots, uint32_t write_rounds, char *log, size_t log_bytes,
+                              char *key, size_t key_bytes);
 int fl_debug_counters(fl_ctx *ctx, uint64_t out4[4]);
 
 
```
